# kyegomez/Tree-Attention-Torch

Hardware: NVIDIA B200
Metric: attention fwd tokens/sec (decode step Sq=1: KV tokens attended per second, whole box, device-timed, max over ranks) at seq=128K (higher is better)
Workload: dtype bf16

## Files before the change

### bench_tools/trace_decode.py

```python
import argparse
import json
import os
import sys

sys.path.insert(0, os.path.dirname(os.path.dirname(os.path.abspath(__file__))))
import torch

from tree_attention_b200 import _build
from tree_attention_b200.ops import local as L


def main():
    ap = argparse.ArgumentParser()
    ap.add_argument("--seq", type=int, nargs="*", default=[16384, 32768, 65536, 131072])
    ap.add_argument("--heads", type=int, default=32)
    ap.add_argument("--dim", type=int, default=128)
    ap.add_argument("--steps", type=int, default=50)
    a = ap.parse_args()
    C = _build.load()
    dev = torch.device("cuda")
    nsm = C.num_sms()
    for S in a.seq:
        g = torch.Generator(device=dev).manual_seed(0)
        q = torch.randn(1, a.heads, 1, a.dim, device=dev, generator=g).bfloat16()
# ... 1 lines not shown
        kvs = [(torch.randn(1, a.heads, S, a.dim, device=dev, generator=g).bfloat16(),
                torch.randn(1, a.heads, S, a.dim, device=dev, generator=g).bfloat16()) for _ in range(min(nbuf, 8))]
        out = torch.empty_like(q)
        res = {"seq": S, "kv_mb": 2 * a.heads * S * a.dim * 2 / 1e6}
        for pdl in (0, 2):
            for i in range(10):
                L.decode_attention(q, *kvs[i % len(kvs)], 0.088, out=out, return_lse=False, pdl=pdl)
            torch.cuda.synchronize()
            e0, e1 = torch.cuda.Event(enable_timing=True), torch.cuda.Event(enable_timing=True)
            e0.record()
            for i in range(a.steps):
                L.decode_attention(q, *kvs[i % len(kvs)], 0.088, out=out, return_lse=False, pdl=pdl)
            e1.record()
            torch.cuda.synchronize()
            res[f"us_per_step_pdl{pdl}"] = e0.elapsed_time(e1) / a.steps * 1e3
        tr = torch.zeros(nsm * 16, dtype=torch.int64, device=dev)
        C.decode_set_trace(tr)
        L.decode_attention(q, *kvs[0], 0.088, out=out, return_lse=False)
        torch.cuda.synchronize()
        tr.zero_()
        e0, e1 = torch.cuda.Event(enable_timing=True), torch.cuda.Event(enable_timing=True)
        e0.record()
        L.decode_attention(q, *kvs[1 % len(kvs)], 0.088, out=out, return_lse=False)
        e1.record()
        torch.cuda.synchronize()
        C.decode_set_trace(None)
        t = tr.view(nsm, 16).cpu().double()
        t = t[t[:, 0] > 0]
        g0 = t[:, 0].min()
        cyc = (t[:, 8] - t[:, 1])
        ns = (t[:, 9] - t[:, 0])
        mhz = float((cyc / ns).median() * 1e3)
        res["traced_kernel_us_event"] = e0.elapsed_time(e1) * 1e3
        res["sm_mhz_from_stamps"] = mhz

        def stat(x):
            x = x.sort().values
            return [round(float(v), 2) for v in (x[0], x[len(x) // 2], x[-1])]

        us = lambda c: c / mhz
        res["cta_start_skew_us(min,med,max)"] = stat((t[:, 0] - g0) / 1e3)
        res["prologue_us"] = stat(us(t[:, 2] - t[:, 1]))
        res["entry_to_first_tma_issue_us"] = stat(us(t[:, 10] - t[:, 1]))
        res["entry_to_first_tile_landed_us"] = stat(us(t[:, 4] - t[:, 1]))
        res["stream_first_tile_to_last_consumed_us"] = stat(us(t[:, 5] - t[:, 4]))
        res["last_finalize_us"] = stat(us(t[:, 6] - t[:, 5]))
        res["drain_us"] = stat(us(t[:, 8] - t[:, 6]))
        res["cta_total_us"] = stat(ns / 1e3)
        res["kernel_span_us(first entry -> last end)"] = float((t[:, 9].max() - g0) / 1e3)
        res["tiles_per_cta"] = stat(t[:, 12])
        res["producer_issue_span_us"] = stat(us(t[:, 11] - t[:, 10]))
        per_tile = us(t[:, 5] - t[:, 4]) / (t[:, 12] - 1).clamp(min=1)
        res["us_per_tile"] = stat(per_tile)
        sw = t[t[:, 14] > 0]
        if len(sw):
            fin = (sw[:, 14].long() & 0xffffffff).double()
            ldq = (sw[:, 14].long() >> 32).double()
            wt = (sw[:, 15].long() & 0xffffffff).double()
            pos = (sw[:, 15].long() >> 32).double()
            res["switch_finalize_us"] = stat(us(fin))
            res["switch_load_q_us"] = stat(us(ldq))
            res["switch_wait_next_tile_us"] = stat(us(wt))
            res["switch_tile_index"] = stat(pos)
            before = us(sw[:, 7] - sw[:, 4]) / pos.clamp(min=1)
            after = us(sw[:, 5] - sw[:, 7]) / (sw[:, 12] - pos).clamp(min=1)
            res["switch_cta_us_per_tile_before"] = stat(before)
            res["switch_cta_us_per_tile_after"] = stat(after)
        if os.environ.get("TRACE_DUMP"):
            torch.save(t, os.path.join(os.environ["TRACE_DUMP"], f"trace_{S}.pt"))
        print(json.dumps(res), flush=True)
        del kvs


if __name__ == "__main__":
    main()
```

### tree_attention_b200/csrc/bindings.cpp

```cpp
#include <ATen/cuda/CUDAContext.h>
#include <c10/cuda/CUDAGuard.h>
#include <pybind11/stl.h>
#include <torch/extension.h>

#include <cstring>

#include "host_utils.h"
#include "kernels.h"

namespace py = pybind11;
using ta::AttnShape;
using ta::CommCtxHost;

namespace {

py::tuple symm_alloc(int64_t nbytes) {
  void* p = nullptr;
  TA_CUDA_CHECK(cudaMalloc(&p, (size_t)nbytes));
  TA_CUDA_CHECK(cudaMemset(p, 0, (size_t)nbytes));
  TA_CUDA_CHECK(cudaDeviceSynchronize());
  cudaIpcMemHandle_t h;
  TA_CUDA_CHECK(cudaIpcGetMemHandle(&h, p));
  return py::make_tuple((int64_t) reinterpret_cast<uintptr_t>(p),
                        py::bytes(reinterpret_cast<const char*>(&h), sizeof(h)));
}
int64_t symm_open(const std::string& handle) {
  if (handle.size() != sizeof(cudaIpcMemHandle_t)) throw std::runtime_error("symm_open: bad handle size");
  cudaIpcMemHandle_t h;
  std::memcpy(&h, handle.data(), sizeof(h));
  void* p = nullptr;
  TA_CUDA_CHECK(cudaIpcOpenMemHandle(&p, h, cudaIpcMemLazyEnablePeerAccess));
  return (int64_t) reinterpret_cast<uintptr_t>(p);
}
void symm_close(int64_t ptr) { TA_CUDA_CHECK(cudaIpcCloseMemHandle(reinterpret_cast<void*>(ptr))); }
void symm_free(int64_t ptr) { TA_CUDA_CHECK(cudaFree(reinterpret_cast<void*>(ptr))); }
void symm_memset(int64_t ptr, int value, int64_t nbytes) {
  TA_CUDA_CHECK(cudaMemsetAsync(reinterpret_cast<void*>(ptr), value, (size_t)nbytes,
                                at::cuda::getCurrentCUDAStream()));
}
std::vector<uint32_t> symm_read_u32(int64_t ptr, int n) {
  std::vector<uint32_t> v(n);
  TA_CUDA_CHECK(cudaMemcpy(v.data(), reinterpret_cast<void*>(ptr), n * sizeof(uint32_t), cudaMemcpyDeviceToHost));
  return v;
}

struct Comm {
  CommCtxHost h;
  Comm(int rank, int world, std::vector<int64_t> data, std::vector<int64_t> flags, int64_t epoch, int64_t status,
       int64_t data_bytes, int64_t flag_bytes, double timeout_s) {
    if (world > ta::kMaxWorldHost) throw std::runtime_error("world size > 16 not supported");
    if ((int)data.size() != world || (int)flags.size() != world) throw std::runtime_error("Comm: pointer table size");
    h.rank = rank;
    h.world = world;
    for (int i = 0; i < world; ++i) {
      h.data[i] = reinterpret_cast<void*>(data[i]);
      h.flags[i] = reinterpret_cast<void*>(flags[i]);
    }
    h.epoch = reinterpret_cast<void*>(epoch);
    h.status = reinterpret_cast<void*>(status);
// ... 3 lines not shown
  }
};

AttnShape make_shape(const at::Tensor& q, const at::Tensor& k, const at::Tensor& v, const at::Tensor& out,
                     double scale, bool causal, int64_t q_pos0, int64_t kv_pos0, bool host_io = false) {
  TORCH_CHECK(k.is_cuda() && v.is_cuda(), "k and v must be CUDA tensors");
  TORCH_CHECK((q.is_cuda() || (host_io && q.is_pinned())) && (out.is_cuda() || (host_io && out.is_pinned())),
              host_io ? "q / out must be CUDA or pinned host tensors" : "tensors must be CUDA");
  TORCH_CHECK(q.dim() == 4 && k.dim() == 4 && v.dim() == 4 && out.dim() == 4, "expected (B, H, S, D) tensors");
  TORCH_CHECK(q.scalar_type() == at::kBFloat16 || q.scalar_type() == at::kHalf, "q must be bf16 or fp16");
  TORCH_CHECK(k.scalar_type() == q.scalar_type() && v.scalar_type() == q.scalar_type() &&
                  out.scalar_type() == q.scalar_type(), "q, k, v, out must share a dtype");
  TORCH_CHECK(q.stride(3) == 1 && k.stride(3) == 1 && v.stride(3) == 1 && out.stride(3) == 1,
              "head_dim must be contiguous");
  TORCH_CHECK(k.sizes() == v.sizes(), "k and v shapes differ");
  TORCH_CHECK(q.size(0) == k.size(0) && q.size(3) == k.size(3), "batch / head_dim mismatch");
  TORCH_CHECK(out.sizes() == q.sizes(), "out must have q's shape");
  AttnShape s;
  s.B = (int)q.size(0); s.Hq = (int)q.size(1); s.Sq = (int)q.size(2); s.D = (int)q.size(3);
  s.Hkv = (int)k.size(1); s.S = (int)k.size(2);
  s.is_bf16 = q.scalar_type() == at::kBFloat16;
  s.softmax_scale = (float)scale;
  s.causal = causal;
  s.q_pos0 = q_pos0; s.kv_pos0 = kv_pos0;
  s.q_sb = q.stride(0); s.q_sh = q.stride(1); s.q_ss = q.stride(2);
  s.k_sb = k.stride(0); s.k_sh = k.stride(1); s.k_ss = k.stride(2);
  s.v_sb = v.stride(0); s.v_sh = v.stride(1); s.v_ss = v.stride(2);
  s.o_sb = out.stride(0); s.o_sh = out.stride(1); s.o_ss = out.stride(2);
  return s;
}

const int* kv_len_ptr(const c10::optional<at::Tensor>& kv_len, const at::Tensor& like) {
  if (!kv_len.has_value()) return nullptr;
  TORCH_CHECK(kv_len->is_cuda() && kv_len->device() == like.device() && kv_len->scalar_type() == at::kInt && kv_len->numel() == 1,
              "kv_len must be a 1-element int32 CUDA tensor on the KV cache's device");
  return kv_len->data_ptr<int>();
}

py::tuple decode_plan(int B, int Hq, int Hkv, int Sq, int S, int D) {
  AttnShape s;
  s.B = B; s.Hq = Hq; s.Hkv = Hkv; s.Sq = Sq; s.S = S; s.D = D;
  int grid, mp, R;
  size_t pf, cf, cfl;
  ta::decode_simt_plan(s, ta::num_sms(), &grid, &mp, &R, &pf, &cf, &cfl);
  return py::make_tuple(grid, mp, R, (int64_t)pf, (int64_t)cf, (int64_t)cfl);
}

void decode_fwd(const at::Tensor& q, const at::Tensor& k, const at::Tensor& v, at::Tensor& out,
                c10::optional<at::Tensor> lse, at::Tensor& part, at::Tensor& tickets, py::object comm, double scale,
                bool causal, int64_t q_pos0, int64_t kv_pos0, int pdl, c10::optional<at::Tensor> kv_len) {
  c10::cuda::CUDAGuard guard(q.device());
  AttnShape s = make_shape(q, k, v, out, scale, causal, q_pos0, kv_pos0);
  TORCH_CHECK(part.scalar_type() == at::kFloat && part.is_contiguous(), "part must be contiguous fp32");
  TORCH_CHECK(tickets.scalar_type() == at::kInt && tickets.numel() >= s.B * s.Hkv + 2, "tickets too small");
  int grid, mp, R;
  size_t pf, cf, cfl;
  ta::decode_simt_plan(s, ta::num_sms(), &grid, &mp, &R, &pf, &cf, &cfl);
  TORCH_CHECK((size_t)part.numel() >= pf, "part workspace too small: need ", pf, " floats");
  float* lse_p = nullptr;
  if (lse.has_value()) {
    TORCH_CHECK(lse->scalar_type() == at::kFloat && lse->is_contiguous() && lse->numel() == (int64_t)s.B * s.Hq * s.Sq,
                "lse must be contiguous fp32 (B, Hq, Sq)");
    lse_p = lse->data_ptr<float>();
  }
  CommCtxHost c;
  if (!comm.is_none()) c = comm.cast<Comm&>().h;
  ta::decode_simt_launch(s, q.data_ptr(), k.data_ptr(), v.data_ptr(), out.data_ptr(), lse_p, part.data_ptr<float>(),
                         reinterpret_cast<uint32_t*>(tickets.data_ptr<int>()), c, ta::num_sms(),
                         at::cuda::getCurrentCUDAStream(), nullptr, nullptr, pdl, kv_len_ptr(kv_len, k));
}

py::tuple attn_fwd_comm_bytes(int B, int Hq, int Sq, int D, int world, int comm_mode) {
  AttnShape s;
  s.B = B; s.Hq = Hq; s.Sq = Sq; s.D = D;
  size_t fb = 0;
  size_t db = ta::attn_fwd_comm_bytes(s, world, &fb, comm_mode);
  return py::make_tuple((int64_t)db, (int64_t)fb);
}

void attn_fwd(const at::Tensor& q, const at::Tensor& k, const at::Tensor& v, at::Tensor& out, at::Tensor& lse,
              double scale, bool causal, int64_t q_pos0, int64_t kv_pos0, py::object comm, int variant, int comm_mode,
              int64_t kv_seg_len, int64_t kv_seg_gap) {
  c10::cuda::CUDAGuard guard(q.device());
  const bool sharded = !comm.is_none() && comm_mode == 2;
  AttnShape s = make_shape(q, k, v, sharded ? q : out, scale, causal, q_pos0, kv_pos0);
  s.kv_seg_len = (int)kv_seg_len; s.kv_seg_gap = kv_seg_gap;
  int64_t sq_out = s.Sq;
  if (sharded) {
    TORCH_CHECK(out.dim() == 4 && out.is_cuda() && out.scalar_type() == q.scalar_type() && out.stride(3) == 1 &&
                    out.size(0) == q.size(0) && out.size(1) == q.size(1) && out.size(3) == q.size(3),
                "sharded out must be (B, Hq, sq_out, D) in q's dtype");
    sq_out = out.size(2);
    const int world = comm.cast<Comm&>().h.world;
    const int64_t num_m = (s.Sq + 127) / 128;
    TORCH_CHECK(sq_out == (num_m + world - 1) / world * 128, "sharded out must have ceil(ceil(Sq/128)/world)*128 rows");
    s.o_sb = out.stride(0); s.o_sh = out.stride(1); s.o_ss = out.stride(2);
  }
  TORCH_CHECK(lse.scalar_type() == at::kFloat && lse.is_contiguous() && lse.numel() == (int64_t)s.B * s.Hq * sq_out,
              "lse must be contiguous fp32 (B, Hq, Sq) [(B, Hq, sq_out) for a sharded output]");
  CommCtxHost c;
  if (!comm.is_none()) c = comm.cast<Comm&>().h;
  TORCH_CHECK(variant == 0 || variant == 1 || variant == 6, "attn_fwd: unknown variant ", variant);
  ta::attn_fwd_launch(s, q.data_ptr(), k.data_ptr(), v.data_ptr(), out.data_ptr(), lse.data_ptr<float>(), c,
                      at::cuda::getCurrentCUDAStream(), variant == 6 ? 1 : 0, comm_mode, (int)sq_out);
}

py::tuple decode_tc_plan(int B, int Hq, int Hkv, int Sq, int S, int D) {
// ... 85 lines not shown
  TORCH_CHECK(ksc.scalar_type() == at::kFloat && vsc.scalar_type() == at::kFloat && ksc.is_contiguous() && vsc.is_contiguous() &&
                  ksc.numel() == k8.size(0) * k8.size(1) * 128 && vsc.numel() == ksc.numel(), "scales must be fp32 (B, Hkv, 128)");
  TORCH_CHECK(q.stride(2) % 8 == 0 || q.size(2) == 1, "q rows must be 16-byte aligned");
  AttnShape s;
  s.B = (int)q.size(0); s.Hq = (int)q.size(1); s.Sq = (int)q.size(2); s.D = 128;
  s.Hkv = (int)k8.size(1); s.S = (int)k8.size(2);
  s.is_bf16 = q.scalar_type() == at::kBFloat16;
  s.softmax_scale = (float)scale; s.causal = causal; s.q_pos0 = q_pos0; s.kv_pos0 = kv_pos0;
  s.q_sb = q.stride(0); s.q_sh = q.stride(1); s.q_ss = q.stride(2);
  s.k_sb = k8.stride(0); s.k_sh = k8.stride(1); s.k_ss = k8.stride(2);
  s.v_sb = v8.stride(0); s.v_sh = v8.stride(1); s.v_ss = v8.stride(2);
  s.o_sb = out.stride(0); s.o_sh = out.stride(1); s.o_ss = out.stride(2);
  int grid, mp, R;
  size_t pf, cb;
  ta::decode_tc_plan(s, ta::num_sms(), &grid, &mp, &R, &pf, &cb);
  TORCH_CHECK((size_t)part.numel() >= pf && tickets.numel() >= s.B * s.Hkv + 2, "workspace too small");
  float* lse_p = lse.has_value() ? lse->data_ptr<float>() : nullptr;
  CommCtxHost c;
  if (!comm.is_none()) c = comm.cast<Comm&>().h;
  if (swap)
    ta::decode_swap_launch(s, q.data_ptr(), k8.data_ptr(), v8.data_ptr(), out.data_ptr(), lse_p, part.data_ptr<float>(),
                           reinterpret_cast<uint32_t*>(tickets.data_ptr<int>()), c, ta::num_sms(), at::cuda::getCurrentCUDAStream(),
                           ksc.data_ptr<float>(), vsc.data_ptr<float>(), nullptr, nullptr, kv_len_ptr(kv_len, k8));
  else
    ta::decode_tc_launch(s, q.data_ptr(), k8.data_ptr(), v8.data_ptr(), out.data_ptr(), lse_p, part.data_ptr<float>(),
                         reinterpret_cast<uint32_t*>(tickets.data_ptr<int>()), c, ta::num_sms(), at::cuda::getCurrentCUDAStream(),
                         ksc.data_ptr<float>(), vsc.data_ptr<float>(), kv_len_ptr(kv_len, k8));
}

void decode_fwd_mx(const at::Tensor& q, const at::Tensor& k8, const at::Tensor& v8, const at::Tensor& ks,
                   const at::Tensor& vs, at::Tensor& out, c10::optional<at::Tensor> lse, at::Tensor& part,
                   at::Tensor& tickets, py::object comm, double scale, bool causal, int64_t q_pos0, int64_t kv_pos0,
                   c10::optional<at::Tensor> kv_len) {
  c10::cuda::CUDAGuard guard(q.device());
  TORCH_CHECK(q.dim() == 4 && k8.dim() == 4 && v8.dim() == 4 && out.sizes() == q.sizes(), "expected (B, H, S, D) tensors");
  TORCH_CHECK(q.scalar_type() == at::kBFloat16 || q.scalar_type() == at::kHalf, "q must be bf16 or fp16");
  TORCH_CHECK(out.scalar_type() == q.scalar_type() && q.stride(3) == 1 && out.stride(3) == 1);
  TORCH_CHECK(k8.scalar_type() == at::kByte && v8.scalar_type() == at::kByte && k8.stride(3) == 1 && v8.stride(3) == 1);
  TORCH_CHECK(k8.sizes() == v8.sizes() && k8.size(3) == 128 && q.size(3) == 128, "mxfp8 decode needs head_dim 128");
  TORCH_CHECK(ks.scalar_type() == at::kByte && vs.scalar_type() == at::kByte && ks.is_contiguous() && vs.is_contiguous() &&
                  ks.numel() == k8.numel() / 32 && vs.numel() == v8.numel() / 32, "scales must be contiguous uint8 (B, Hkv, S, 4)");
  AttnShape s;
  s.B = (int)q.size(0); s.Hq = (int)q.size(1); s.Sq = (int)q.size(2); s.D = 128;
  s.Hkv = (int)k8.size(1); s.S = (int)k8.size(2);
  s.is_bf16 = q.scalar_type() == at::kBFloat16;
  s.softmax_scale = (float)scale; s.causal = causal; s.q_pos0 = q_pos0; s.kv_pos0 = kv_pos0;
  s.q_sb = q.stride(0); s.q_sh = q.stride(1); s.q_ss = q.stride(2);
  s.k_sb = k8.stride(0); s.k_sh = k8.stride(1); s.k_ss = k8.stride(2);
  s.v_sb = v8.stride(0); s.v_sh = v8.stride(1); s.v_ss = v8.stride(2);
  s.o_sb = out.stride(0); s.o_sh = out.stride(1); s.o_ss = out.stride(2);
  int grid, mp, R;
  size_t pf, cf, cfl;
  ta::decode_simt_plan(s, ta::num_sms(), &grid, &mp, &R, &pf, &cf, &cfl);
  TORCH_CHECK((size_t)part.numel() >= pf && tickets.numel() >= s.B * s.Hkv + 2, "workspace too small");
  float* lse_p = lse.has_value() ? lse->data_ptr<float>() : nullptr;
  CommCtxHost c;
  if (!comm.is_none()) c = comm.cast<Comm&>().h;
  ta::decode_simt_launch(s, q.data_ptr(), k8.data_ptr(), v8.data_ptr(), out.data_ptr(), lse_p, part.data_ptr<float>(),
                         reinterpret_cast<uint32_t*>(tickets.data_ptr<int>()), c, ta::num_sms(),
                         at::cuda::getCurrentCUDAStream(), reinterpret_cast<const uint32_t*>(ks.data_ptr()),
                         reinterpret_cast<const uint32_t*>(vs.data_ptr()), 0, kv_len_ptr(kv_len, k8));
}

struct DecodeStep {
  ta::PreparedLaunch launches[3];
  bool has[3] = {false, false, false};
  std::vector<at::Tensor> keep;
  py::object comm_keep;
  c10::Device device;
  int kernels_per_step = 1;
  std::string impl;

  explicit DecodeStep(c10::Device d) : device(d) {}

  void launch(int pdl) {
    c10::cuda::CUDAGuard guard(device);
    if (pdl < 0 || pdl > 2 || !has[pdl]) pdl = 0;
    launches[pdl].run(at::cuda::getCurrentCUDAStream());
  }
};

void* io_ptr(const at::Tensor& t) {
  if (t.is_cuda()) return t.data_ptr();
  void* d = nullptr;
  const cudaError_t e = cudaHostGetDevicePointer(&d, t.data_ptr(), 0);
  TORCH_CHECK(e == cudaSuccess && d != nullptr, "pinned host tensor is not mapped into the device address space: ", cudaGetErrorString(e));
  return d;
}

std::shared_ptr<DecodeStep> decode_step(const std::string& impl, const at::Tensor& q, const at::Tensor& k, const at::Tensor& v,
                                        at::Tensor& out, c10::optional<at::Tensor> lse, at::Tensor& part, at::Tensor& tickets,
                                        py::object comm, double scale, bool causal, int64_t q_pos0, int64_t kv_pos0,
                                        c10::optional<at::Tensor> kv_len) {
  c10::cuda::CUDAGuard guard(k.device());
  AttnShape s = make_shape(q, k, v, out, scale, causal, q_pos0, kv_pos0, true);
  TORCH_CHECK(part.scalar_type() == at::kFloat && part.is_contiguous(), "part must be contiguous fp32");
  TORCH_CHECK(tickets.scalar_type() == at::kInt && tickets.numel() >= s.B * s.Hkv + 2, "tickets too small");
  float* lse_p = nullptr;
  if (lse.has_value()) {
    TORCH_CHECK(lse->scalar_type() == at::kFloat && lse->is_contiguous() && lse->numel() == (int64_t)s.B * s.Hq * s.Sq,
                "lse must be contiguous fp32 (B, Hq, Sq)");
    lse_p = lse->data_ptr<float>();
  }
  CommCtxHost c;
  if (!comm.is_none()) c = comm.cast<Comm&>().h;
  auto st = std::make_shared<DecodeStep>(k.device());
  st->impl = impl;
  st->comm_keep = comm;
  st->keep = {q, k, v, out, part, tickets};
  if (lse.has_value()) st->keep.push_back(*lse);
  if (kv_len.has_value()) st->keep.push_back(*kv_len);
  const int* kvl = kv_len_ptr(kv_len, k);
  uint32_t* tk = reinterpret_cast<uint32_t*>(tickets.data_ptr<int>());
  if (impl == "simt") {
    int grid, mp, R;
    size_t pf, cf, cfl;
    ta::decode_simt_plan(s, ta::num_sms(), &grid, &mp, &R, &pf, &cf, &cfl);
    TORCH_CHECK((size_t)part.numel() >= pf, "part workspace too small: need ", pf, " floats");
    for (int pdl = 0; pdl < 3; ++pdl) {
      st->launches[pdl] = ta::decode_simt_prepare(s, io_ptr(q), k.data_ptr(), v.data_ptr(), io_ptr(out), lse_p,
                                                  part.data_ptr<float>(), tk, c, ta::num_sms(), nullptr, nullptr, pdl, kvl);
      st->has[pdl] = true;
    }
    st->kernels_per_step = (int)st->launches[0].passes.size();
  } else if (impl == "swap" || impl == "tc") {
    int grid, mp, R;
    size_t pf, cb;
    ta::decode_tc_plan(s, ta::num_sms(), &grid, &mp, &R, &pf, &cb);
    TORCH_CHECK((size_t)part.numel() >= pf, "part workspace too small: need ", pf, " floats");
    TORCH_CHECK(q.stride(2) % 8 == 0 || q.size(2) == 1, "q rows must be 16-byte aligned");
    st->launches[0] = impl == "swap"
                          ? ta::decode_swap_prepare(s, io_ptr(q), k.data_ptr(), v.data_ptr(), io_ptr(out), lse_p,
                                                    part.data_ptr<float>(), tk, c, ta::num_sms(), nullptr, nullptr, nullptr, nullptr, kvl)
                          : ta::decode_tc_prepare(s, io_ptr(q), k.data_ptr(), v.data_ptr(), io_ptr(out), lse_p,
                                                  part.data_ptr<float>(), tk, c, ta::num_sms(), nullptr, nullptr, kvl);
    st->has[0] = true;
  } else {
    TORCH_CHECK(false, "decode_step: impl must be 'simt', 'swap' or 'tc'");
  }
  return st;
}

py::tuple quant_mxfp8(const at::Tensor& x) {
  c10::cuda::CUDAGuard guard(x.device());
  TORCH_CHECK(x.is_cuda() && x.is_contiguous() && x.size(-1) % 32 == 0, "x must be contiguous with last dim % 32 == 0");
  int dt = x.scalar_type() == at::kBFloat16 ? 0 : x.scalar_type() == at::kHalf ? 1 : 2;
  TORCH_CHECK(dt != 2 || x.scalar_type() == at::kFloat, "x must be bf16, fp16 or fp32");
  auto q = at::empty(x.sizes(), x.options().dtype(at::kByte));
  auto sizes = x.sizes().vec();
  sizes.back() /= 32;
  auto sc = at::empty(sizes, x.options().dtype(at::kByte));
  ta::quant_mxfp8_launch(x.data_ptr(), dt, q.data_ptr<uint8_t>(), sc.data_ptr<uint8_t>(), x.numel() / 32,
                         at::cuda::getCurrentCUDAStream());
  return py::make_tuple(q, sc);
}

py::tuple quant_mxfp8_seq(const at::Tensor& x) {
  c10::cuda::CUDAGuard guard(x.device());
  TORCH_CHECK(x.is_cuda() && x.is_contiguous() && x.dim() == 4 && x.size(3) % 32 == 0, "x must be contiguous (B, H, S, D), D % 32 == 0");
  int dt = x.scalar_type() == at::kBFloat16 ? 0 : x.scalar_type() == at::kHalf ? 1 : 2;
  TORCH_CHECK(dt != 2 || x.scalar_type() == at::kFloat, "x must be bf16, fp16 or fp32");
  const int64_t B = x.size(0), H = x.size(1), S = x.size(2), D = x.size(3), T = (S + 127) / 128;
  auto q = at::empty(x.sizes(), x.options().dtype(at::kByte));
  auto sc = at::empty({B, H, T, D, 4}, x.options().dtype(at::kByte));
  ta::quant_mxfp8_seq_launch(x.data_ptr(), dt, q.data_ptr<uint8_t>(), sc.data_ptr<uint8_t>(), B * H, (int)S, (int)D,
                             at::cuda::getCurrentCUDAStream());
  return py::make_tuple(q, sc);
}

void mxfp8_seq_append(at::Tensor& data, at::Tensor& sc, const at::Tensor& x, int64_t position) {
  c10::cuda::CUDAGuard guard(data.device());
// ... 117 lines not shown
  m.def("decode_fwd", &decode_fwd, py::arg("q"), py::arg("k"), py::arg("v"), py::arg("out"), py::arg("lse"), py::arg("part"),
        py::arg("tickets"), py::arg("comm"), py::arg("scale"), py::arg("causal"), py::arg("q_pos0"), py::arg("kv_pos0"),
        py::arg("pdl") = 0, py::arg("kv_len") = py::none());
  m.def("decode_fwd_mx", &decode_fwd_mx, py::arg("q"), py::arg("k8"), py::arg("v8"), py::arg("ks"), py::arg("vs"), py::arg("out"),
        py::arg("lse"), py::arg("part"), py::arg("tickets"), py::arg("comm"), py::arg("scale"), py::arg("causal"),
        py::arg("q_pos0"), py::arg("kv_pos0"), py::arg("kv_len") = py::none());
  m.def("decode_set_trace", [](c10::optional<at::Tensor> t) {
    if (!t.has_value()) { ta::decode_simt_set_trace(nullptr); return; }
    TORCH_CHECK(t->is_cuda() && t->scalar_type() == at::kLong && t->is_contiguous() && t->numel() >= 16 * ta::num_sms());
    ta::decode_simt_set_trace(reinterpret_cast<unsigned long long*>(t->data_ptr<int64_t>()));
  });
  m.def("decode_tc_plan", &decode_tc_plan);
  m.def("decode_tc_fwd", &decode_tc_fwd, py::arg("q"), py::arg("k"), py::arg("v"), py::arg("out"), py::arg("lse"), py::arg("part"),
        py::arg("tickets"), py::arg("comm"), py::arg("scale"), py::arg("causal"), py::arg("q_pos0"), py::arg("kv_pos0"),
        py::arg("swap"), py::arg("kv_len") = py::none());
  m.def("decode_tc_fwd8", &decode_tc_fwd8, py::arg("q"), py::arg("k8"), py::arg("v8"), py::arg("ksc"), py::arg("vsc"), py::arg("out"),
        py::arg("lse"), py::arg("part"), py::arg("tickets"), py::arg("comm"), py::arg("scale"), py::arg("causal"),
        py::arg("q_pos0"), py::arg("kv_pos0"), py::arg("swap"), py::arg("kv_len") = py::none());
  m.def("decode_mx_tc_fwd", &decode_mx_tc_fwd, py::arg("q"), py::arg("k8"), py::arg("v8"), py::arg("k_sf"), py::arg("v_sf"),
        py::arg("out"), py::arg("lse"), py::arg("part"), py::arg("tickets"), py::arg("comm"), py::arg("scale"), py::arg("causal"),
        py::arg("q_pos0"), py::arg("kv_pos0"), py::arg("kv_len") = py::none());
  py::class_<DecodeStep, std::shared_ptr<DecodeStep>>(m, "DecodeStep")
      .def("launch", &DecodeStep::launch, py::arg("pdl") = 0)
      .def_readonly("kernels_per_step", &DecodeStep::kernels_per_step)
      .def_readonly("impl", &DecodeStep::impl);
  m.def("decode_step", &decode_step, py::arg("impl"), py::arg("q"), py::arg("k"), py::arg("v"), py::arg("out"), py::arg("lse"),
        py::arg("part"), py::arg("tickets"), py::arg("comm"), py::arg("scale"), py::arg("causal"), py::arg("q_pos0"),
        py::arg("kv_pos0"), py::arg("kv_len") = py::none());
  m.def("quant_mxfp8", &quant_mxfp8);
  m.def("quant_mxfp8_seq", &quant_mxfp8_seq);
  m.def("mxfp8_seq_append", &mxfp8_seq_append);
  m.def("dequant_mxfp8", &dequant_mxfp8);
  m.def("attn_fwd", &attn_fwd, py::arg("q"), py::arg("k"), py::arg("v"), py::arg("out"), py::arg("lse"), py::arg("scale"),
        py::arg("causal"), py::arg("q_pos0"), py::arg("kv_pos0"), py::arg("comm"), py::arg("variant") = 0, py::arg("comm_mode") = 1,
        py::arg("kv_seg_len") = 0, py::arg("kv_seg_gap") = 0);
  m.def("attn_fwd_comm_bytes", &attn_fwd_comm_bytes, py::arg("B"), py::arg("Hq"), py::arg("Sq"), py::arg("D"), py::arg("world"),
        py::arg("comm_mode") = 1);
  m.def("attn_fwd_phase_cycles", []() { unsigned long long c[5]; ta::attn_fwd_phase_cycles(c); return py::make_tuple(c[0], c[1], c[2], c[3], c[4]); });
  m.def("attn_bwd", &attn_bwd);
  m.def("symm_allreduce", &symm_allreduce);
  m.def("symm_allreduce_sizes", &symm_allreduce_sizes);
  m.def("combine", &combine);
  m.def("umma_probe", &umma_probe);
  m.def("umma_bs_probe", &umma_bs_probe, py::arg("a8"), py::arg("b8"), py::arg("sfa"), py::arg("sfb"), py::arg("c"),
        py::arg("a_mn_major") = false);
  m.def("umma_2cta_probe", [](const at::Tensor& a, const at::Tensor& b, at::Tensor& c) {
    c10::cuda::CUDAGuard guard(a.device());
    TORCH_CHECK(a.scalar_type() == at::kBFloat16 && b.scalar_type() == at::kBFloat16 && c.scalar_type() == at::kFloat);
    TORCH_CHECK(a.is_contiguous() && b.is_contiguous() && c.is_contiguous() && a.size(0) == 256 && a.size(1) == 64 &&
                b.size(0) == 128 && b.size(1) == 64 && c.size(0) == 256 && c.size(1) == 128);
    ta::umma_2cta_probe_launch(a.data_ptr(), b.data_ptr(), c.data_ptr<float>(), 128, at::cuda::getCurrentCUDAStream());
  });
  m.def("num_sms", []() { return ta::num_sms(); });
  m.def("decode_split_for", [](int B, int Hkv, int S, int ncta) {
    AttnShape s{};
    s.B = B; s.Hkv = Hkv; s.Hq = Hkv; s.Sq = 1; s.S = S; s.D = 128;
    int g = 0, mp = 0;
    ta::decode_split(B * Hkv, S, ncta, &g, &mp);
    return py::make_tuple(g, mp);
  });
  m.def("tmem_ld_bw_probe", [](int warps, int iters) { return ta::tmem_ld_bw_probe(warps, iters, at::cuda::getCurrentCUDAStream()); });
}
```

### tree_attention_b200/csrc/common.cuh

```cuda
#pragma once
#include <cuda.h>
#include <cuda_bf16.h>
#include <cuda_fp16.h>
#include <cuda_runtime.h>
#include <stdint.h>
#include <stdio.h>

namespace ta {

#ifndef TA_SPIN_TIMEOUT_NS
#define TA_SPIN_TIMEOUT_NS 4000000000ull
#endif

constexpr int kMaxWorld = 16;

__device__ __forceinline__ uint32_t smem_u32(const void* p) {
  return static_cast<uint32_t>(__cvta_generic_to_shared(p));
}
__device__ __forceinline__ uint64_t globaltimer_ns() {
  uint64_t t;
  asm volatile("mov.u64 %0, %%globaltimer;" : "=l"(t));
  return t;
}
__device__ __forceinline__ uint32_t lane_id() { return threadIdx.x & 31; }
// ... 62 lines not shown
__device__ __forceinline__ float bf16lo(uint32_t w) { return __uint_as_float(w << 16); }
__device__ __forceinline__ float bf16hi(uint32_t w) { return __uint_as_float(w & 0xffff0000u); }
__device__ __forceinline__ uint32_t pack_bf16x2(float lo, float hi) {
  uint32_t r;
  asm("cvt.rn.bf16x2.f32 %0, %1, %2;" : "=r"(r) : "f"(hi), "f"(lo));
  return r;
}
__device__ __forceinline__ uint32_t pack_f16x2(float lo, float hi) {
  uint32_t r;
  asm("cvt.rn.f16x2.f32 %0, %1, %2;" : "=r"(r) : "f"(hi), "f"(lo));
  return r;
}
__device__ __forceinline__ float f16lo(uint32_t w) {
  return __half2float(__ushort_as_half(static_cast<unsigned short>(w & 0xffffu)));
}
__device__ __forceinline__ float f16hi(uint32_t w) {
  return __half2float(__ushort_as_half(static_cast<unsigned short>(w >> 16)));
}

__device__ __forceinline__ uint64_t pack_f32x2(float a, float b) {
  uint64_t r;
  asm("mov.b64 %0, {%1, %2};" : "=l"(r) : "f"(a), "f"(b));
  return r;
}
__device__ __forceinline__ void unpack_f32x2(uint64_t v, float& a, float& b) {
  asm("mov.b64 {%0, %1}, %2;" : "=f"(a), "=f"(b) : "l"(v));
}
__device__ __forceinline__ uint64_t fma2_f32x2(uint64_t a, uint64_t b, uint64_t c) {
  uint64_t d;
  asm("fma.rn.f32x2 %0, %1, %2, %3;" : "=l"(d) : "l"(a), "l"(b), "l"(c));
  return d;
}
__device__ __forceinline__ uint64_t add2_f32x2(uint64_t a, uint64_t b) {
  uint64_t d;
  asm("add.rn.f32x2 %0, %1, %2;" : "=l"(d) : "l"(a), "l"(b));
  return d;
}

__device__ __forceinline__ void mbar_init(uint64_t* bar, uint32_t count) {
  asm volatile("mbarrier.init.shared::cta.b64 [%0], %1;" ::"r"(smem_u32(bar)), "r"(count) : "memory");
}
__device__ __forceinline__ void fence_mbar_init() {
  asm volatile("fence.mbarrier_init.release.cluster;" ::: "memory");
}
__device__ __forceinline__ void fence_proxy_async_smem() {
  asm volatile("fence.proxy.async.shared::cta;" ::: "memory");
}
__device__ __forceinline__ void mbar_arrive(uint64_t* bar) {
  asm volatile("mbarrier.arrive.shared::cta.b64 _, [%0];" ::"r"(smem_u32(bar)) : "memory");
}
__device__ __forceinline__ void mbar_arrive_expect_tx(uint64_t* bar, uint32_t bytes) {
  asm volatile("mbarrier.arrive.expect_tx.shared::cta.b64 _, [%0], %1;" ::"r"(smem_u32(bar)), "r"(bytes)
               : "memory");
}
__device__ __forceinline__ bool mbar_try_wait(uint64_t* bar, uint32_t parity) {
  uint32_t ok;
  asm volatile(
      "{\n\t.reg .pred P;\n\t"
      "mbarrier.try_wait.parity.shared::cta.b64 P, [%1], %2;\n\t"
      "selp.u32 %0, 1, 0, P;\n\t}"
      : "=r"(ok)
      : "r"(smem_u32(bar)), "r"(parity)
      : "memory");
  return ok != 0;
}
__device__ __forceinline__ void mbar_wait(uint64_t* bar, uint32_t parity) {
  if (mbar_try_wait(bar, parity)) return;
  uint64_t t0 = globaltimer_ns();
  uint32_t it = 0;
  while (!mbar_try_wait(bar, parity)) {
    if ((++it & 0x3ffu) == 0 && globaltimer_ns() - t0 > TA_SPIN_TIMEOUT_NS) {
      printf("[tree_attention] mbarrier wait timeout block=(%d,%d) thread=%d bar=%u parity=%u\n",
             blockIdx.x, blockIdx.y, threadIdx.x, smem_u32(bar), parity);
      __trap();
    }
  }
}

__device__ __forceinline__ void tma_prefetch_desc(const CUtensorMap* m) {
  asm volatile("prefetch.tensormap [%0];" ::"l"(reinterpret_cast<uint64_t>(m)) : "memory");
}
__device__ __forceinline__ void tma_load_4d(void* smem_dst, const CUtensorMap* map, uint64_t* bar,
                                            int c0, int c1, int c2, int c3) {
  asm volatile(
      "cp.async.bulk.tensor.4d.shared::cluster.global.mbarrier::complete_tx::bytes [%0], [%1, {%3, %4, %5, %6}], [%2];"
      ::"r"(smem_u32(smem_dst)), "l"(reinterpret_cast<uint64_t>(map)), "r"(smem_u32(bar)), "r"(c0), "r"(c1),
      "r"(c2), "r"(c3)
      : "memory");
}
__device__ __forceinline__ void tma_load_2d(void* smem_dst, const CUtensorMap* map, uint64_t* bar,
                                            int c0, int c1) {
  asm volatile(
      "cp.async.bulk.tensor.2d.shared::cluster.global.mbarrier::complete_tx::bytes [%0], [%1, {%3, %4}], [%2];"
      ::"r"(smem_u32(smem_dst)), "l"(reinterpret_cast<uint64_t>(map)), "r"(smem_u32(bar)), "r"(c0), "r"(c1)
      : "memory");
}
__device__ __forceinline__ void tma_store_4d(const CUtensorMap* map, const void* smem_src, int c0, int c1,
                                             int c2, int c3) {
  asm volatile(
      "cp.async.bulk.tensor.4d.global.shared::cta.bulk_group [%0, {%2, %3, %4, %5}], [%1];"
      ::"l"(reinterpret_cast<uint64_t>(map)), "r"(smem_u32(smem_src)), "r"(c0), "r"(c1), "r"(c2), "r"(c3)
      : "memory");
}
__device__ __forceinline__ void tma_store_commit() { asm volatile("cp.async.bulk.commit_group;" ::: "memory"); }
template <int N>
__device__ __forceinline__ void tma_store_wait_read() {
// ... 213 lines not shown
```

### tree_attention_b200/csrc/decode_comm.cuh

```cuda
#pragma once
#include "common.cuh"
#include "kernels.h"

namespace ta {
namespace dcomm {

constexpr int kTileKeys = 128;
constexpr int kPartChunk = 8;

__device__ __forceinline__ float ninf() { return __int_as_float(0xff800000); }

struct Geom {
  int S;
  int tph;
  int total;
  int tiles_q, tiles_rem;
};

__device__ __forceinline__ Geom make_geom(int cap, const int* kv_len, int BH, int ncta) {
  Geom g;
  int s = cap;
  if (kv_len != nullptr) s = max(0, min(cap, *reinterpret_cast<const volatile int*>(kv_len)));
  g.S = s;
  g.tph = max(1, (s + kTileKeys - 1) / kTileKeys);
  g.total = BH * g.tph;
  g.tiles_q = g.total / ncta;
  g.tiles_rem = g.total - g.tiles_q * ncta;
  return g;
}
__device__ __forceinline__ int cta_lo(const Geom& g, int c) { return c * g.tiles_q + min(c, g.tiles_rem); }
__device__ __forceinline__ int cta_of_tile(const Geom& g, int t) {
  const int big = g.tiles_rem * (g.tiles_q + 1);
  return t < big ? t / (g.tiles_q + 1) : g.tiles_rem + (t - big) / max(g.tiles_q, 1);
}

__device__ __forceinline__ void ll_store_sys(uint64_t* w, float v, uint32_t tag) {
  const uint64_t x = ((uint64_t)tag << 32) | (uint64_t)__float_as_uint(v);
  asm volatile("st.relaxed.sys.global.u64 [%0], %1;" ::"l"(w), "l"(x) : "memory");
}
__device__ __forceinline__ uint64_t ll_load_sys(const uint64_t* w) {
  uint64_t r;
  asm volatile("ld.relaxed.sys.global.u64 %0, [%1];" : "=l"(r) : "l"(w) : "memory");
  return r;
}
__device__ __forceinline__ void ll_store_gpu(uint64_t* w, float v, uint32_t tag) {
  const uint64_t x = ((uint64_t)tag << 32) | (uint64_t)__float_as_uint(v);
  asm volatile("st.relaxed.gpu.global.u64 [%0], %1;" ::"l"(w), "l"(x) : "memory");
}
__device__ __forceinline__ uint64_t ll_load_gpu(const uint64_t* w) {
  uint64_t r;
  asm volatile("ld.relaxed.gpu.global.u64 %0, [%1];" : "=l"(r) : "l"(w) : "memory");
  return r;
}
__device__ __forceinline__ uint32_t ll_tag(uint64_t w) { return (uint32_t)(w >> 32); }
__device__ __forceinline__ float ll_val(uint64_t w) { return __uint_as_float((uint32_t)w); }

static __device__ __noinline__ uint64_t ll_spin_sys(const uint64_t* w, uint32_t tag, unsigned long long timeout_ns) {
  const uint64_t t0 = globaltimer_ns();
  uint32_t it = 0;
  uint64_t out;
  while (true) {
    out = ll_load_sys(w);
    if (ll_tag(out) == tag) break;
    if ((++it & 0x3fu) == 0 && globaltimer_ns() - t0 > timeout_ns) break;
  }
  return out;
}
static __device__ __noinline__ uint64_t ll_spin_gpu(const uint64_t* w, uint32_t tag) {
  const uint64_t t0 = globaltimer_ns();
  uint32_t it = 0;
  uint64_t out;
  while (true) {
    out = ll_load_gpu(w);
    if (ll_tag(out) == tag) break;
    if ((++it & 0x3fu) == 0 && globaltimer_ns() - t0 > TA_SPIN_TIMEOUT_NS) {
      printf("[tree_attention] split-merge wait timeout block=%d thread=%d tag=%u\n", blockIdx.x, threadIdx.x, tag);
      __trap();
    }
  }
  return out;
}

constexpr int kTagShift = 12;

__device__ __forceinline__ uint32_t launch_tag(unsigned long long* ctr) {
  const unsigned long long inc = blockIdx.x == 0 ? (unsigned long long)((1u << kTagShift) - (gridDim.x - 1)) : 1ull;
  const unsigned long long old = atomicAdd(ctr, inc);
  return (uint32_t)(old >> kTagShift) + 1u;
}

struct Tail {
  const CommCtx* comm;
  uint64_t* part;
  int max_parts;
  int BH;
  int R;
  int rows_valid;
  uint32_t wtag;
  uint32_t ctag;
  Geom geo;
  int* pending;
  int max_pending;
  uint64_t* stamps;
};

template <int D>
__device__ __forceinline__ uint64_t* part_ptr(const Tail& t, int x, int pidx) {
  return t.part + ((size_t)x * t.max_parts + pidx) * (size_t)(t.R * (D + 2));
}
template <int D>
__device__ __forceinline__ uint64_t* word_ptr(const Tail& t, int dst, int src, int x) {
  return reinterpret_cast<uint64_t*>(t.comm->data[dst]) +
         ((size_t)((t.ctag & 1) * t.comm->world + src) * t.BH + x) * (size_t)(t.R * (D + 2));
}
__device__ __forceinline__ void head_parts(const Geom& g, int x, int cta, int& nparts, int& pidx) {
  const int first_cta = cta_of_tile(g, x * g.tph);
  nparts = cta_of_tile(g, (x + 1) * g.tph - 1) - first_cta + 1;
  pidx = cta - first_cta;
}

template <int D>
__device__ __forceinline__ void merge_parts(const Tail& t, int x, int nparts, int r, int d, float& o_norm, float& lse2) {
  const size_t pstride = (size_t)t.R * (D + 2);
  const uint64_t* base = part_ptr<D>(t, x, 0) + (size_t)r * (D + 2);
  float M = ninf(), acc = 0.f, L = 0.f;
  for (int q0 = 0; q0 < nparts; q0 += kPartChunk) {
    uint64_t wa[kPartChunk], wm[kPartChunk], wl[kPartChunk];
#pragma unroll
    for (int i = 0; i < kPartChunk; ++i) {
      if (q0 + i < nparts) {
        const uint64_t* pp = base + (size_t)(q0 + i) * pstride;
        wa[i] = ll_load_gpu(pp + d); wm[i] = ll_load_gpu(pp + D); wl[i] = ll_load_gpu(pp + D + 1);
      }
    }
    float m[kPartChunk], a[kPartChunk], l[kPartChunk];
    float Mn = M;
#pragma unroll
    for (int i = 0; i < kPartChunk; ++i) {
      m[i] = ninf(); a[i] = 0.f; l[i] = 0.f;
      if (q0 + i < nparts) {
        const uint64_t* pp = base + (size_t)(q0 + i) * pstride;
        if (ll_tag(wa[i]) != t.wtag) wa[i] = ll_spin_gpu(pp + d, t.wtag);
        if (ll_tag(wm[i]) != t.wtag) wm[i] = ll_spin_gpu(pp + D, t.wtag);
        if (ll_tag(wl[i]) != t.wtag) wl[i] = ll_spin_gpu(pp + D + 1, t.wtag);
        a[i] = ll_val(wa[i]); m[i] = ll_val(wm[i]); l[i] = ll_val(wl[i]);
        Mn = fmaxf(Mn, m[i]);
      }
    }
    const float Ms = (Mn == ninf()) ? 0.f : Mn;
    const float sc0 = fast_exp2(M - Ms);
    acc *= sc0; L *= sc0;
#pragma unroll
    for (int i = 0; i < kPartChunk; ++i) {
      const float sc = fast_exp2(m[i] - Ms);
      acc = fmaf(a[i], sc, acc);
      L = fmaf(l[i], sc, L);
    }
    M = Mn;
  }
  const float Ms = (M == ninf()) ? 0.f : M;
  o_norm = L > 0.f ? acc / L : 0.f;
  lse2 = L > 0.f ? Ms + fast_log2(L) : ninf();
}

template <int D>
__device__ __forceinline__ void publish(const Tail& t, int x, int r, int d, float o_norm, float lse2) {
  const int world = t.comm->world;
#pragma unroll 4
  for (int dst = 0; dst < world; ++dst) {
    uint64_t* wp = word_ptr<D>(t, dst, t.comm->rank, x) + r * (D + 2);
    ll_store_sys(wp + d, o_norm, t.ctag);
    if (d == 0) ll_store_sys(wp + D, lse2, t.ctag);
  }
}

template <int D, int RB>
__device__ __forceinline__ bool gather_rows(const Tail& t, int x, int r0, int nr, int d, float (&o_norm)[RB],
                                            float (&lse2)[RB], int& bad_src) {
  constexpr int kSrcChunk = RB >= 4 ? 4 : 8;
  const int world = t.comm->world;
  const size_t src_stride = (size_t)t.BH * t.R * (D + 2);
  const uint64_t* w0 = word_ptr<D>(t, t.comm->rank, 0, x);
  float m_run[RB], num[RB], den[RB];
#pragma unroll
  for (int i = 0; i < RB; ++i) { m_run[i] = ninf(); num[i] = 0.f; den[i] = 0.f; }
  bool ok = true;
  for (int s0 = 0; s0 < world; s0 += kSrcChunk) {
    uint64_t lw[RB][kSrcChunk], vw[RB][kSrcChunk];
#pragma unroll
    for (int i = 0; i < RB; ++i) {
#pragma unroll
      for (int s = 0; s < kSrcChunk; ++s) {
        if (i < nr && s0 + s < world) {
          const uint64_t* wr = w0 + (size_t)(s0 + s) * src_stride + (size_t)(r0 + i) * (D + 2);
          lw[i][s] = ll_load_sys(wr + D);
          vw[i][s] = ll_load_sys(wr + d);
        }
// ... 24 lines not shown
        for (int s = 0; s < kSrcChunk; ++s) {
          const float w = fast_exp2(ls[s] - ms);
          num[i] = fmaf(w, vs[s], num[i]);
          den[i] += w;
        }
        m_run[i] = mc;
      }
    }
  }
#pragma unroll
  for (int i = 0; i < RB; ++i) {
    const float ms = (m_run[i] == ninf()) ? 0.f : m_run[i];
    o_norm[i] = den[i] > 0.f ? num[i] / den[i] : 0.f;
    lse2[i] = den[i] > 0.f ? ms + fast_log2(den[i]) : ninf();
  }
  return ok;
}

template <int D, int NT, int RB, typename StoreOut>
__device__ __noinline__ void combine_ranks(const Tail& t, int x, int tid, int bar_id, StoreOut& store_out) {
  static_assert(NT % D == 0, "thread count must be a multiple of head_dim");
  constexpr int NG = NT / D;
  const int d = tid % D, g = tid / D;
  uint64_t t_got = 0;
  for (int r0 = g * RB; r0 < t.rows_valid; r0 += NG * RB) {
    const int nr = min(RB, t.rows_valid - r0);
    float o_norm[RB], lse2[RB];
    int bad_src = -1;
    const bool ok = gather_rows<D, RB>(t, x, r0, nr, d, o_norm, lse2, bad_src);
    if (tid == 0 && r0 == 0) t_got = globaltimer_ns();
    if (!ok) {
      t.comm->status[0] = kCommTimeout; t.comm->status[1] = x; t.comm->status[2] = bad_src; t.comm->status[3] = t.ctag;
    }
#pragma unroll
    for (int i = 0; i < RB; ++i) {
      if (i < nr) {
        const float nan = __int_as_float(0x7fc00000);
        store_out(x, r0 + i, d, ok ? o_norm[i] : nan, ok ? lse2[i] : nan);
      }
    }
  }
  if (tid == 0 && t.stamps[1] != 0) {
    const uint64_t t_done = globaltimer_ns(), t_publish = t.stamps[1], t_cta0 = t.stamps[0];
    atomicMax(t.comm->status + 10, (uint32_t)min((unsigned long long)(t_got - t_publish), 0xffffffffull));
    atomicMax(t.comm->status + 11, (uint32_t)min((unsigned long long)(t_done - t_publish), 0xffffffffull));
    atomicMax(t.comm->status + 12, (uint32_t)min((unsigned long long)(t_publish - t_cta0), 0xffffffffull));
  }
}

template <int D, int NT, typename StoreOut>
__device__ __noinline__ void merge_head(const Tail& t, int x, int tid, StoreOut& store_out) {
  static_assert(NT % D == 0, "thread count must be a multiple of head_dim");
  constexpr int NG = NT / D;
  int nparts, pidx;
  head_parts(t.geo, x, blockIdx.x, nparts, pidx);
  const int world = t.comm->world;
  const int d = tid % D;
  for (int r = tid / D; r < t.rows_valid; r += NG) {
    float o_norm, lse2;
    merge_parts<D>(t, x, nparts, r, d, o_norm, lse2);
    if (world == 1) store_out(x, r, d, o_norm, lse2);
    else if (!t.comm->skip_publish) publish<D>(t, x, r, d, o_norm, lse2);
  }
}

template <int D, int NT, int RB, typename StoreOut>
__device__ __forceinline__ void segment_done(const Tail& t, int x, int seg_end_tile, int& n_pend, int tid, int bar_id,
                                             StoreOut& store_out) {
  if (seg_end_tile != (x + 1) * t.geo.tph) return;
  if (n_pend >= t.max_pending) {
    printf("[tree_attention] pending-merge list overflow block=%d head=%d\n", blockIdx.x, x);
    __trap();
  }
  if (tid == 0) t.pending[n_pend] = x;
  ++n_pend;
}

template <int D, int NT, int RB, typename StoreOut>
__device__ __forceinline__ void drain(const Tail& t, int n_pend, int tid, int bar_id, StoreOut& store_out) {
  named_bar_sync(bar_id, NT);
  for (int i = 0; i < n_pend; ++i) merge_head<D, NT>(t, t.pending[i], tid, store_out);
  if (t.comm->world <= 1 || n_pend == 0) return;
  if (tid == 0) t.stamps[1] = globaltimer_ns();
  named_bar_sync(bar_id, NT);
  for (int i = 0; i < n_pend; ++i) combine_ranks<D, NT, RB>(t, t.pending[i], tid, bar_id, store_out);
}

inline CommCtx to_device_ctx(const CommCtxHost& h) {
  CommCtx c;
  c.rank = h.rank;
  c.world = h.world;
  for (int i = 0; i < kMaxWorld; ++i) {
    c.data[i] = reinterpret_cast<float*>(h.data[i]);
    c.flags[i] = reinterpret_cast<uint32_t*>(h.flags[i]);
  }
  c.epoch = reinterpret_cast<uint32_t*>(h.epoch);
  c.status = reinterpret_cast<uint32_t*>(h.status);
  c.timeout_ns = h.timeout_ns;
  c.skip_publish = h.skip_publish;
  return c;
}

}
}
```

### tree_attention_b200/csrc/decode_simt.cu

```cuda
#include "common.cuh"
#include "decode_comm.cuh"
#include "host_utils.h"
#include "kernels.h"

namespace ta {

namespace {

constexpr int kTileRows = 128;
constexpr int kConsumerWarps = 8;
constexpr int kConsumerThreads = kConsumerWarps * 32;
constexpr int kThreads = kConsumerThreads + 32;
constexpr int kRowsPerWarp = kTileRows / kConsumerWarps;
constexpr int kMaxPending = 64;

struct DecodeParams {
  const void* q;
  void* out;
  float* lse;
  const uint32_t* kscale;
  const uint32_t* vscale;
  uint64_t* part;
  unsigned long long* wctr;
  const int* kv_len;
  int B, Hq, Hkv, G, Sq, S;
  int rows_valid;
  int r_base;
  float scale_log2;
  int causal;
  long long q_pos0, kv_pos0;
  long long q_sb, q_sh, q_ss, o_sb, o_sh, o_ss;
  int max_parts;
  unsigned long long* trace;
  int pdl;
  CommCtx comm;
};

template <int D, bool KV8>
struct SmemLayout {
  static constexpr int kElem = KV8 ? 1 : 2;
  static constexpr int kAtoms = D * kElem / 128;
  static constexpr int kTensorBytes = kTileRows * D * kElem;
  static constexpr int kStageBytes = 2 * kTensorBytes;
  static constexpr int kStages = (D * kElem == 256) ? 3 : 6;
  static constexpr int kPsPerWarp = KV8 ? 4 : 1;
};

template <int D, int R, bool KV8>
constexpr size_t smem_bytes() {
  using L = SmemLayout<D, KV8>;
  return 1024  + size_t(L::kStages) * L::kStageBytes +
         sizeof(float) * (2 * R * D + kConsumerWarps * L::kPsPerWarp * R * kRowsPerWarp +
                          (R <= 2 ? 2 : 1) * kConsumerWarps * R * (D + 4)) +
         sizeof(int) * (kMaxPending + 8) + sizeof(uint64_t) * (2 * L::kStages + 2);
}

template <bool BF16>
__device__ __forceinline__ void cvt8(const uint4& w, float (&f)[8]) {
  if constexpr (BF16) {
    f[0] = bf16lo(w.x); f[1] = bf16hi(w.x); f[2] = bf16lo(w.y); f[3] = bf16hi(w.y);
    f[4] = bf16lo(w.z); f[5] = bf16hi(w.z); f[6] = bf16lo(w.w); f[7] = bf16hi(w.w);
  } else {
    f[0] = f16lo(w.x); f[1] = f16hi(w.x); f[2] = f16lo(w.y); f[3] = f16hi(w.y);
    f[4] = f16lo(w.z); f[5] = f16hi(w.z); f[6] = f16lo(w.w); f[7] = f16hi(w.w);
  }
}
template <bool BF16>
__device__ __forceinline__ float cvt1(uint16_t h) {
  if constexpr (BF16) return __uint_as_float(uint32_t(h) << 16);
  else return __half2float(__ushort_as_half(h));
}
template <bool BF16>
__device__ __forceinline__ uint16_t to16(float f) {
  if constexpr (BF16) return __bfloat16_as_ushort(__float2bfloat16_rn(f));
  else return __half_as_ushort(__float2half_rn(f));
}

__device__ __forceinline__ float neg_inf() { return __int_as_float(0xff800000); }

template <int D, int R, bool BF16, bool KV8>
__global__ void __launch_bounds__(kThreads, 1)
decode_simt_kernel(const __grid_constant__ CUtensorMap kmap, const __grid_constant__ CUtensorMap vmap,
                   const __grid_constant__ DecodeParams p) {
  using L = SmemLayout<D, KV8>;
  constexpr int NS = L::kStages;
  constexpr int EPL = D / 32;
  extern __shared__ uint8_t smem_raw[];
  uint8_t* smem = reinterpret_cast<uint8_t*>((reinterpret_cast<uintptr_t>(smem_raw) + 1023) & ~uintptr_t(1023));
  uint8_t* stage_base = smem;
  float* q_s = reinterpret_cast<float*>(smem + size_t(NS) * L::kStageBytes);
  float* p_s = q_s + 2 * R * D;
  float* merge_s = p_s + kConsumerWarps * L::kPsPerWarp * R * kRowsPerWarp;
  constexpr int kMergeBufs = R <= 2 ? 2 : 1;
  int* pending = reinterpret_cast<int*>(merge_s + kMergeBufs * kConsumerWarps * R * (D + 4));
  int* s_misc = pending + kMaxPending;
  uint64_t* full_bar = reinterpret_cast<uint64_t*>(s_misc + 8);
  uint64_t* empty_bar = full_bar + NS;
  uint64_t* stamps = empty_bar + NS;

  const int tid = threadIdx.x;
  const int warp = tid >> 5;
  const int lane = tid & 31;
  const int cta = blockIdx.x;
  const int world = p.comm.world;
  unsigned long long* trc = p.trace ? p.trace + (size_t)cta * 16 : nullptr;
  if (trc && tid == 0) {
    trc[0] = globaltimer_ns(); trc[1] = clock64();
    uint32_t smid;
    asm volatile("mov.u32 %0, %%smid;" : "=r"(smid));
    trc[13] = smid; trc[14] = 0; trc[15] = 0;
  }

  if (tid == 0) {
    for (int i = 0; i < NS; ++i) {
      mbar_init(&full_bar[i], 1);
      mbar_init(&empty_bar[i], kConsumerWarps);
    }
    fence_mbar_init();
    s_misc[0] = 0; s_misc[1] = 0; s_misc[6] = 0;
  }
  if (warp == kConsumerWarps && lane == 0) {
    tma_prefetch_desc(&kmap);
    tma_prefetch_desc(&vmap);
  }
  __syncthreads();
  if (trc && tid == 0) trc[2] = clock64();

  if (p.pdl) asm volatile("griddepcontrol.launch_dependents;" ::: "memory");
  const int BH = p.B * p.Hkv;
  const long long q_pos_max = p.q_pos0 + p.Sq - 1;

  auto tile_visible = [&](int j) -> bool {
    return !p.causal || (p.kv_pos0 + (long long)j * kTileRows <= q_pos_max);
  };

  if (warp == kConsumerWarps) {
    if (lane == 0) {
      if (p.pdl == 1) asm volatile("griddepcontrol.wait;" ::: "memory");
      const dcomm::Geom geo = dcomm::make_geom(p.S, p.kv_len, BH, gridDim.x);
      const int t_lo = dcomm::cta_lo(geo, cta), t_hi = dcomm::cta_lo(geo, cta + 1);
      int stage = 0, issued = 0;
      uint32_t phase = 0;
      bool tags_done = false;
      auto fetch_tags = [&]() {
        if (p.pdl == 2) asm volatile("griddepcontrol.wait;" ::: "memory");
        const uint32_t wtag = dcomm::launch_tag(p.wctr);
        const uint32_t ctag = world > 1 ? dcomm::launch_tag(reinterpret_cast<unsigned long long*>(p.comm.epoch)) : 0u;
        volatile int* sm = s_misc;
        sm[4] = (int)wtag; sm[5] = (int)ctag;
        __threadfence_block();
        sm[6] = 1;
        tags_done = true;
      };
      for (int t = t_lo; t < t_hi; ++t) {
        const int x = t / geo.tph, j = t - x * geo.tph;
        if (!tile_visible(j)) continue;
        const int b = x / p.Hkv, h = x - b * p.Hkv;
        if (issued == NS && !tags_done) fetch_tags();
        mbar_wait(&empty_bar[stage], phase ^ 1);
        if (trc && issued == 0) trc[10] = clock64();
        mbar_arrive_expect_tx(&full_bar[stage], L::kStageBytes);
        uint8_t* ks = stage_base + size_t(stage) * L::kStageBytes;
        uint8_t* vs = ks + L::kTensorBytes;
#pragma unroll
        for (int a = 0; a < L::kAtoms; ++a) {
          tma_load_4d(ks + a * (kTileRows * 128), &kmap, &full_bar[stage], a * (128 / L::kElem), j * kTileRows, h, b);
          tma_load_4d(vs + a * (kTileRows * 128), &vmap, &full_bar[stage], a * (128 / L::kElem), j * kTileRows, h, b);
        }
        ++issued;
        if (++stage == NS) { stage = 0; phase ^= 1; }
      }
      if (!tags_done) fetch_tags();
      if (trc) { trc[11] = clock64(); trc[12] = (unsigned long long)issued; }
    }
    return;
  }

  if (p.pdl) asm volatile("griddepcontrol.wait;" ::: "memory");
  if (trc && tid == 0) trc[3] = clock64();
  const dcomm::Geom geo = dcomm::make_geom(p.S, p.kv_len, BH, gridDim.x);
  const int t_lo = dcomm::cta_lo(geo, cta), t_hi = dcomm::cta_lo(geo, cta + 1);
  constexpr int RB = R;
  if (tid == 0) { stamps[0] = globaltimer_ns(); stamps[1] = 0; }
  auto make_tail = [&]() {
    dcomm::Tail tl;
    volatile int* sm = s_misc;
    while (sm[6] == 0) { }
    tl.comm = &p.comm; tl.part = p.part; tl.max_parts = p.max_parts; tl.BH = BH;
    tl.R = R; tl.rows_valid = p.rows_valid; tl.wtag = (uint32_t)sm[4]; tl.ctag = (uint32_t)sm[5]; tl.geo = geo;
    tl.pending = pending; tl.max_pending = kMaxPending; tl.stamps = stamps;
    return tl;
  };
  const int r16 = lane & 15;
  const int half = lane >> 4;
  float m_run[R], l_run[R], o_acc[R][EPL];
  int cur_x = -1;
  int stage = 0;
  uint32_t phase = 0;

  auto reset_state = [&]() {
#pragma unroll
    for (int r = 0; r < R; ++r) {
      m_run[r] = neg_inf();
      l_run[r] = 0.f;
#pragma unroll
      for (int e = 0; e < EPL; ++e) o_acc[r][e] = 0.f;
    }
  };

  auto load_q = [&](int x, int buf) {
    const int b = x / p.Hkv, h = x - b * p.Hkv;
    for (int idx = tid; idx < R * D; idx += kConsumerThreads) {
      const int r = idx / D, d = idx - r * D;
      float val = 0.f;
      if (r < p.rows_valid) {
        const int rr = p.r_base + r;
        const int g = rr / p.Sq, i = rr - g * p.Sq;
        const uint16_t* qp = reinterpret_cast<const uint16_t*>(p.q) + (long long)b * p.q_sb +
                             (long long)(h * p.G + g) * p.q_sh + (long long)i * p.q_ss + d;
        val = cvt1<BF16>(*qp) * p.scale_log2;
      }
      if constexpr (KV8) reinterpret_cast<__half*>(q_s + buf * R * D)[idx] = __float2half_rn(val);
      else q_s[buf * R * D + idx] = val;
    }
  };
  const int x_first = t_lo / geo.tph;
  if (t_lo < t_hi) {
    load_q(x_first, 0);
    if ((x_first + 1) * geo.tph < t_hi) load_q(x_first + 1, 1);
  }
  named_bar_sync(1, kConsumerThreads);
  const float* q_cur = q_s;
  uint32_t wtag = 0;
  int n_fin = 0;
  int n_pend = 0;

  auto store_out = [&](int x, int r, int d, float o_norm, float lse2) {
    const int b = x / p.Hkv, h = x - b * p.Hkv;
    const int rr = p.r_base + r;
    const int g = rr / p.Sq, i = rr - g * p.Sq;
    uint16_t* op = reinterpret_cast<uint16_t*>(p.out) + (long long)b * p.o_sb + (long long)(h * p.G + g) * p.o_sh +
                   (long long)i * p.o_ss + d;
    *op = to16<BF16>(o_norm);
    if (d == 0 && p.lse != nullptr)
      p.lse[((long long)b * p.Hq + (h * p.G + g)) * p.Sq + i] = lse2 * 0.6931471805599453f;
  };

  auto finalize_segment = [&](int x) {
    float* mbuf = merge_s + (kMergeBufs == 2 ? (n_fin & 1) : 0) * (kConsumerWarps * R * (D + 4));
    ++n_fin;
#pragma unroll
    for (int r = 0; r < R; ++r) {
      float lt = l_run[r];
      lt += __shfl_xor_sync(0xffffffffu, lt, 8);
      lt += __shfl_xor_sync(0xffffffffu, lt, 4);
      lt += __shfl_xor_sync(0xffffffffu, lt, 2);
      lt += __shfl_xor_sync(0xffffffffu, lt, 1);
      float* ms = mbuf + (warp * R + r) * (D + 4);
#pragma unroll
      for (int e = 0; e < EPL; ++e) ms[lane * EPL + e] = o_acc[r][e];
      if (lane == 0) { ms[D] = m_run[r]; ms[D + 1] = lt; }
    }
    named_bar_sync(1, kConsumerThreads);
    if (wtag == 0) {
      volatile int* sm = s_misc;
      while (sm[6] == 0) { }
      wtag = (uint32_t)sm[4];
    }
    int nparts, pidx;
    dcomm::head_parts(geo, x, cta, nparts, pidx);
    uint64_t* my_part = p.part + ((size_t)x * p.max_parts + pidx) * (size_t)(R * (D + 2));
    for (int idx = tid; idx < R * D; idx += kConsumerThreads) {
      const int r = idx / D, d = idx - r * D;
      float M = neg_inf();
#pragma unroll
      for (int w = 0; w < kConsumerWarps; ++w) M = fmaxf(M, mbuf[(w * R + r) * (D + 4) + D]);
      const float Ms = (M == neg_inf()) ? 0.f : M;
      float acc = 0.f, Lsum = 0.f;
#pragma unroll
      for (int w = 0; w < kConsumerWarps; ++w) {
        const float* ms = mbuf + (w * R + r) * (D + 4);
        const float sc = fast_exp2(ms[D] - Ms);
        acc = fmaf(ms[d], sc, acc);
        Lsum = fmaf(ms[D + 1], sc, Lsum);
      }
      dcomm::ll_store_gpu(my_part + r * (D + 2) + d, acc, wtag);
      if (d == 0) {
        dcomm::ll_store_gpu(my_part + r * (D + 2) + D, M, wtag);
        dcomm::ll_store_gpu(my_part + r * (D + 2) + D + 1, Lsum, wtag);
      }
    }
    if (min(t_hi, (x + 1) * geo.tph) == (x + 1) * geo.tph) {
      if (tid == 0) pending[n_pend] = x;
      ++n_pend;
    }
    if constexpr (kMergeBufs == 1) named_bar_sync(1, kConsumerThreads);
  };

  [[maybe_unused]] uint32_t nxt_ksc = 0, nxt_vsc = 0;
  [[maybe_unused]] auto fetch_scales = [&](int tt) {
    if constexpr (KV8) {
      if (tt < t_hi) {
        const int xx = tt / geo.tph, jj = tt - xx * geo.tph;
        const long long srow = (long long)xx * p.S + min((long long)jj * kTileRows + warp * kRowsPerWarp + (lane & 15), (long long)p.S - 1);
        nxt_ksc = __ldg(p.kscale + srow);
        nxt_vsc = __ldg(p.vscale + srow);
      }
    }
  };
  fetch_scales(t_lo);

  const uint32_t stage_a = smem_u32(stage_base);
  const uint32_t ps_a = smem_u32(p_s);
  [[maybe_unused]] uint32_t k_off[D / 16];
  [[maybe_unused]] uint32_t v_sw[8];
  [[maybe_unused]] uint32_t q_off[D / 16];
  if constexpr (!KV8) {
    const int row = warp * kRowsPerWarp + r16;
#pragma unroll
    for (int c = 0; c < D / 16; ++c) {
      const int cg = half * (D / 16) + c;
      const int atom = cg >> 3, cia = cg & 7;
      k_off[c] = uint32_t(atom * (kTileRows * 128) + row * 128 + ((cia ^ (row & 7)) << 4));
      q_off[c] = uint32_t(cg * 8 * 4);
    }
    const int c0 = lane * EPL;
    const int atom = (c0 * 2) >> 7, inner = (c0 * 2) & 127;
    const int chunk = inner >> 4, off = inner & 15;
#pragma unroll
    for (int k7 = 0; k7 < 8; ++k7)
      v_sw[k7] = uint32_t(L::kTensorBytes + atom * (kTileRows * 128) + off + ((chunk ^ k7) << 4) + (warp * kRowsPerWarp) * 128);
  }

  for (int t = t_lo; t < t_hi; ++t) {
    const int x = t / geo.tph, j = t - x * geo.tph;
    [[maybe_unused]] const uint32_t ksc_word = nxt_ksc;
    [[maybe_unused]] const uint32_t vsc_cur = nxt_vsc;
    fetch_scales(t + 1);
    bool switched = false;
    long long ts0 = 0, ts1 = 0, ts2 = 0;
    if (x != cur_x) {
      switched = cur_x >= 0;
      ts0 = clock64();
      if (cur_x >= 0) finalize_segment(cur_x);
      ts1 = clock64();
      const int rel = x - x_first;
      if (rel >= 2) {
        load_q(x, rel & 1);
        named_bar_sync(1, kConsumerThreads);
      }
      q_cur = q_s + (rel & 1) * R * D;
      reset_state();
      cur_x = x;
      ts2 = clock64();
    }
    if (!tile_visible(j)) continue;
    mbar_wait(&full_bar[stage], phase);
    if (trc && tid == 0 && t == t_lo) trc[4] = clock64();
    if (trc && tid == 0 && switched) {
      trc[14] = (unsigned long long)(ts1 - ts0) | ((unsigned long long)(ts2 - ts1) << 32);
      trc[15] = (unsigned long long)(clock64() - ts2) | ((unsigned long long)(t - t_lo) << 32);
      trc[7] = (unsigned long long)ts0;
    }
    const uint8_t* ks = stage_base + size_t(stage) * L::kStageBytes;
    const uint8_t* vs = ks + L::kTensorBytes;

    const int row = warp * kRowsPerWarp + r16;
    float s_sum[R];
    [[maybe_unused]] uint32_t vsc_word = 0;
    if constexpr (!KV8) {
      const uint32_t ks_a = stage_a + uint32_t(stage) * L::kStageBytes;
      const uint32_t q_a = smem_u32(q_cur);
      uint64_t acc2[R][2];
#pragma unroll
      for (int r = 0; r < R; ++r) { acc2[r][0] = 0ull; acc2[r][1] = 0ull; }
#pragma unroll
      for (int c = 0; c < D / 16; ++c) {
        const uint4 kw = ld_shared_v4u(ks_a + k_off[c]);
        uint64_t k2[4];
        if constexpr (BF16) {
          k2[0] = pack_f32x2(bf16lo(kw.x), bf16hi(kw.x)); k2[1] = pack_f32x2(bf16lo(kw.y), bf16hi(kw.y));
          k2[2] = pack_f32x2(bf16lo(kw.z), bf16hi(kw.z)); k2[3] = pack_f32x2(bf16lo(kw.w), bf16hi(kw.w));
        } else {
          k2[0] = pack_f32x2(f16lo(kw.x), f16hi(kw.x)); k2[1] = pack_f32x2(f16lo(kw.y), f16hi(kw.y));
          k2[2] = pack_f32x2(f16lo(kw.z), f16hi(kw.z)); k2[3] = pack_f32x2(f16lo(kw.w), f16hi(kw.w));
        }
#pragma unroll
        for (int r = 0; r < R; ++r) {
          uint64_t q01, q23, q45, q67;
          ld_shared_v2u64(q_a + uint32_t(r * D * 4) + q_off[c], q01, q23);
          ld_shared_v2u64(q_a + uint32_t(r * D * 4) + q_off[c] + 16, q45, q67);
          acc2[r][0] = fma2_f32x2(k2[0], q01, acc2[r][0]);
          acc2[r][1] = fma2_f32x2(k2[1], q23, acc2[r][1]);
          acc2[r][0] = fma2_f32x2(k2[2], q45, acc2[r][0]);
          acc2[r][1] = fma2_f32x2(k2[3], q67, acc2[r][1]);
        }
      }
#pragma unroll
      for (int r = 0; r < R; ++r) {
        float a0, a1, a2, a3;
        unpack_f32x2(acc2[r][0], a0, a1);
        unpack_f32x2(acc2[r][1], a2, a3);
        s_sum[r] = (a0 + a1) + (a2 + a3);
      }
    } else {
      vsc_word = vsc_cur;
#pragma unroll
      for (int r = 0; r < R; ++r) s_sum[r] = 0.f;
#pragma unroll
      for (int c = 0; c < 4; ++c) {
        const int cg = half * 4 + c;
        const uint4 kw = *reinterpret_cast<const uint4*>(ks + row * 128 + ((cg ^ (row & 7)) << 4));
        uint32_t kh[8];
        const uint32_t kw4[4] = {kw.x, kw.y, kw.z, kw.w};
#pragma unroll
// ... 80 lines not shown
        for (int u = 0; u < 4; ++u) {
          const int vrow = warp * kRowsPerWarp + jj + u;
          const uint32_t w = *reinterpret_cast<const uint32_t*>(vs + vrow * 128 + ((chunk ^ (vrow & 7)) << 4) + off);
          uint32_t h0, h1;
          asm("cvt.rn.f16x2.e4m3x2 %0, %1;" : "=r"(h0) : "h"((uint16_t)(w & 0xffffu)));
          asm("cvt.rn.f16x2.e4m3x2 %0, %1;" : "=r"(h1) : "h"((uint16_t)(w >> 16)));
          const float2 v01 = __half22float2(*reinterpret_cast<const __half2*>(&h0));
          const float2 v23 = __half22float2(*reinterpret_cast<const __half2*>(&h1));
#pragma unroll
          for (int r = 0; r < R; ++r) {
            const float pp = (u == 0) ? pr[r].x : (u == 1) ? pr[r].y : (u == 2) ? pr[r].z : pr[r].w;
            o_acc[r][0] = fmaf(pp, v01.x, o_acc[r][0]);
            o_acc[r][1] = fmaf(pp, v01.y, o_acc[r][1]);
            o_acc[r][2] = fmaf(pp, v23.x, o_acc[r][2]);
            o_acc[r][3] = fmaf(pp, v23.y, o_acc[r][3]);
          }
        }
      }
    } else
    {
      const uint32_t vs_a = stage_a + uint32_t(stage) * L::kStageBytes;
#pragma unroll
      for (int jj = 0; jj < kRowsPerWarp; jj += 4) {
        float4 pr[R];
#pragma unroll
        for (int r = 0; r < R; ++r) pr[r] = ld_shared_v4f(ps_a + uint32_t(((warp * R + r) * kRowsPerWarp + jj) * 4));
#pragma unroll
        for (int u = 0; u < 4; ++u) {
          const uint32_t va = vs_a + v_sw[(jj + u) & 7] + uint32_t((jj + u) * 128);
          float vf[EPL];
          if constexpr (EPL == 4) {
            const uint2 w = ld_shared_v2u(va);
            if constexpr (BF16) { vf[0] = bf16lo(w.x); vf[1] = bf16hi(w.x); vf[2] = bf16lo(w.y); vf[3] = bf16hi(w.y); }
            else { vf[0] = f16lo(w.x); vf[1] = f16hi(w.x); vf[2] = f16lo(w.y); vf[3] = f16hi(w.y); }
          } else {
            const uint32_t w = ld_shared_u32(va);
            if constexpr (BF16) { vf[0] = bf16lo(w); vf[1] = bf16hi(w); }
            else { vf[0] = f16lo(w); vf[1] = f16hi(w); }
          }
#pragma unroll
          for (int r = 0; r < R; ++r) {
            const float pp = (u == 0) ? pr[r].x : (u == 1) ? pr[r].y : (u == 2) ? pr[r].z : pr[r].w;
#pragma unroll
            for (int e = 0; e < EPL; ++e) o_acc[r][e] = fmaf(pp, vf[e], o_acc[r][e]);
          }
        }
      }
    }
    __syncwarp();
    if (lane == 0) mbar_arrive(&empty_bar[stage]);
    if (++stage == NS) { stage = 0; phase ^= 1; }
  }
  if (trc && tid == 0) trc[5] = clock64();
  if (cur_x >= 0) finalize_segment(cur_x);
  if (trc && tid == 0) trc[6] = clock64();

  const dcomm::Tail tail = make_tail();
  dcomm::drain<D, kConsumerThreads, RB>(tail, n_pend, tid, 1, store_out);
  if (trc && tid == 0) { trc[8] = clock64(); trc[9] = globaltimer_ns(); }
}

template <int D, int R, bool BF16, bool KV8>
std::function<void(cudaStream_t)> make_pass(const CUtensorMap& kmap, const CUtensorMap& vmap, const DecodeParams& p, int grid) {
  auto kern = decode_simt_kernel<D, R, BF16, KV8>;
  constexpr size_t smem = smem_bytes<D, R, KV8>();
  static bool configured = false;
  if (!configured) {
    TA_CUDA_CHECK(cudaFuncSetAttribute(kern, cudaFuncAttributeMaxDynamicSharedMemorySize, (int)smem));
    configured = true;
  }
  return [kern, kmap, vmap, p, grid](cudaStream_t stream) {
    cudaLaunchConfig_t cfg{};
    cfg.gridDim = dim3(grid);
    cfg.blockDim = dim3(kThreads);
    cfg.dynamicSmemBytes = smem_bytes<D, R, KV8>();
    cfg.stream = stream;
    cudaLaunchAttribute attr[1];
    attr[0].id = cudaLaunchAttributeProgrammaticStreamSerialization;
    attr[0].val.programmaticStreamSerializationAllowed = 1;
    cfg.attrs = attr;
    cfg.numAttrs = p.pdl ? 1 : 0;
    TA_CUDA_CHECK(cudaLaunchKernelEx(&cfg, kern, kmap, vmap, p));
  };
}

int pick_rows(int total_rows) { return total_rows >= 4 ? 4 : (total_rows >= 2 ? 2 : 1); }

unsigned long long* g_decode_trace = nullptr;

}

void decode_simt_set_trace(unsigned long long* buf) { g_decode_trace = buf; }

void decode_split(int BH, int cap, int ncta, int* grid, int* max_parts) {
  const int tph = std::max(1, (cap + kTileRows - 1) / kTileRows);
  const long long total = (long long)BH * tph;
  const int g = (int)std::min<long long>(ncta, total);
  const int mp = std::min<long long>(g, (2LL * g + BH - 1) / BH + 1);
  *grid = g;
  *max_parts = std::max(mp, 1);
}

void decode_simt_plan(const AttnShape& s, int nsm, int* grid, int* max_parts, int* rows_per_pass,
                      size_t* part_floats, size_t* comm_floats, size_t* comm_flags) {
  const int BH = s.B * s.Hkv;
  decode_split(BH, s.S, nsm, grid, max_parts);
  const int R = pick_rows((s.Hq / s.Hkv) * s.Sq);
  *rows_per_pass = R;
  *part_floats = (size_t)BH * *max_parts * R * (s.D + 2) * 2;
  *comm_floats = (size_t)2 * kMaxWorldHost * BH * R * (s.D + 2) * 2;
  *comm_flags = (size_t)2 * kMaxWorldHost * BH;
}

PreparedLaunch decode_simt_prepare(const AttnShape& s, const void* q, const void* k, const void* v, void* out, float* lse,
                                   float* part, uint32_t* tickets, const CommCtxHost& comm, int nsm,
                                   const uint32_t* kscale, const uint32_t* vscale, int pdl, const int* kv_len) {
  if ((reinterpret_cast<uintptr_t>(part) | reinterpret_cast<uintptr_t>(tickets)) & 7)
    throw std::runtime_error("decode_simt: workspace must be 8-byte aligned");
  const bool kv8 = kscale != nullptr;
  if (s.D != 64 && s.D != 128) throw std::runtime_error("decode_simt: head_dim must be 64 or 128");
  if (kv8 && s.D != 128) throw std::runtime_error("decode_simt(mxfp8): head_dim must be 128");
  if (s.Hq % s.Hkv != 0) throw std::runtime_error("decode_simt: Hq must be a multiple of Hkv");
  if (s.S <= 0) throw std::runtime_error("decode_simt: the KV shard must have capacity for at least one row");
  int grid, max_parts, R;
  size_t pf, cf, cfl;
  decode_simt_plan(s, nsm, &grid, &max_parts, &R, &pf, &cf, &cfl);
  const int G = s.Hq / s.Hkv;
  const int total_rows = G * s.Sq;
  if ((long long)s.B * s.Hkv / grid + 2 > kMaxPending)
    throw std::runtime_error("decode_simt: batch x kv-heads too large for one launch (split the batch)");
  if (comm.world > 1) {
    const size_t need_data = (size_t)2 * comm.world * s.B * s.Hkv * R * (s.D + 2) * 8;
    if (need_data > comm.data_bytes)
      throw std::runtime_error("decode_simt: symmetric buffer too small for this problem");
  }
  const int eb = kv8 ? 1 : 2;
  CUtensorMap kmap = make_tmap_bhsd(k, eb, s.B, s.Hkv, s.S, s.D, s.k_sb, s.k_sh, s.k_ss, 128 / eb, kTileRows,
                                    CU_TENSOR_MAP_SWIZZLE_128B);
  CUtensorMap vmap = make_tmap_bhsd(v, eb, s.B, s.Hkv, s.S, s.D, s.v_sb, s.v_sh, s.v_ss, 128 / eb, kTileRows,
                                    CU_TENSOR_MAP_SWIZZLE_128B);
  DecodeParams p;
  p.kscale = kscale; p.vscale = vscale; p.pdl = pdl; p.kv_len = kv_len; p.trace = g_decode_trace;
  p.q = q; p.out = out; p.lse = lse;
  p.part = reinterpret_cast<uint64_t*>(part); p.wctr = reinterpret_cast<unsigned long long*>(tickets);
  p.B = s.B; p.Hq = s.Hq; p.Hkv = s.Hkv; p.G = G; p.Sq = s.Sq; p.S = s.S;
  p.scale_log2 = s.softmax_scale * 1.4426950408889634f;
  p.causal = s.causal; p.q_pos0 = s.q_pos0; p.kv_pos0 = s.kv_pos0;
  p.q_sb = s.q_sb; p.q_sh = s.q_sh; p.q_ss = s.q_ss; p.o_sb = s.o_sb; p.o_sh = s.o_sh; p.o_ss = s.o_ss;
  p.max_parts = max_parts;
  p.comm = dcomm::to_device_ctx(comm);
  PreparedLaunch pl;
  for (int r_base = 0; r_base < total_rows; r_base += R) {
    p.r_base = r_base;
    p.rows_valid = std::min(R, total_rows - r_base);
#define TA_PASS(DD, RR, KV)                                                                       \
  pl.passes.push_back(s.is_bf16 ? make_pass<DD, RR, true, KV>(kmap, vmap, p, grid)               \
                                : make_pass<DD, RR, false, KV>(kmap, vmap, p, grid));
    if (kv8) {
      if (R == 4) { TA_PASS(128, 4, true) } else if (R == 2) { TA_PASS(128, 2, true) } else { TA_PASS(128, 1, true) }
    } else if (s.D == 128) {
      if (R == 4) { TA_PASS(128, 4, false) } else if (R == 2) { TA_PASS(128, 2, false) } else { TA_PASS(128, 1, false) }
    } else {
      if (R == 4) { TA_PASS(64, 4, false) } else if (R == 2) { TA_PASS(64, 2, false) } else { TA_PASS(64, 1, false) }
    }
#undef TA_PASS
  }
  return pl;
}

void decode_simt_launch(const AttnShape& s, const void* q, const void* k, const void* v, void* out, float* lse,
                        float* part, uint32_t* tickets, const CommCtxHost& comm, int nsm, cudaStream_t stream,
                        const uint32_t* kscale, const uint32_t* vscale, int pdl, const int* kv_len) {
  decode_simt_prepare(s, q, k, v, out, lse, part, tickets, comm, nsm, kscale, vscale, pdl, kv_len).run(stream);
}

}
```

### tree_attention_b200/csrc/decode_swap_sm100.cu

```cuda
#include "common.cuh"
#include "decode_comm.cuh"
#include "host_utils.h"
#include "kernels.h"

namespace ta {
namespace {

constexpr int kSwN = 16;
constexpr int kSwKV = 128;
constexpr int kSwD = 128;
constexpr int kSwThreads = 192;
constexpr int kSmx = 128;
constexpr int kSwMaxPending = 32;
constexpr float kSwRescale = 8.0f;
constexpr uint32_t kSfK = 96;
constexpr uint32_t kSfV = 104;
constexpr uint32_t kSfQ = 112;
constexpr uint32_t kSfP = 116;
constexpr uint32_t kSfOne = 0x7f7f7f7fu;

struct DecodeSwParams {
  const void* q;
  void* out;
  float* lse;
// ... 25 lines not shown
  static constexpr int kPBytes = kSwN * kSwKV * kElem;
  static constexpr int kPAtoms = kSwKV * kElem / 128;
  static constexpr int kStages = KV8 ? 6 : 3;
  static constexpr size_t kTotal = 1024 + size_t(2 * kStages) * kTileBytes + kQBytes + 2 * kPBytes + 2048 + 1024;
};

__device__ __forceinline__ float sw_ninf() { return __int_as_float(0xff800000); }
template <bool BF16>
__device__ __forceinline__ uint16_t sw_to16(float f) {
  if constexpr (BF16) return __bfloat16_as_ushort(__float2bfloat16_rn(f));
  else return __half_as_ushort(__float2half_rn(f));
}
__device__ __forceinline__ int sw_f2ord(float f) { const int i = __float_as_int(f); return i ^ ((i >> 31) & 0x7fffffff); }
__device__ __forceinline__ float sw_ord2f(int i) { return __int_as_float(i ^ ((i >> 31) & 0x7fffffff)); }

template <bool BF16, bool KV8, bool MX>
__global__ void __launch_bounds__(kSwThreads, 1)
decode_swap_kernel(const __grid_constant__ CUtensorMap kmap, const __grid_constant__ CUtensorMap vmap,
                   const __grid_constant__ DecodeSwParams p) {
  using SM = SwSmem<KV8>;
  constexpr int D = kSwD;
  constexpr int NS = SM::kStages;
  constexpr int EPA = 128 / SM::kElem;
  constexpr int KSTEP = 32 / SM::kElem;
  extern __shared__ uint8_t smem_raw[];
  uint8_t* smem = reinterpret_cast<uint8_t*>((reinterpret_cast<uintptr_t>(smem_raw) + 1023) & ~uintptr_t(1023));
  uint8_t* k_s = smem;
  uint8_t* v_s = k_s + NS * SM::kTileBytes;
  uint8_t* q_s = v_s + NS * SM::kTileBytes;
  uint8_t* p_s = q_s + SM::kQBytes;
  float* xch = reinterpret_cast<float*>(p_s + 2 * SM::kPBytes);
  float* red_s = xch + 2 * 4 * kSwN;
  uint64_t* bars = reinterpret_cast<uint64_t*>(red_s + 4 * kSwN);
  uint64_t* q_ready = bars;
  uint64_t* k_full = bars + 1;
  uint64_t* k_empty = k_full + NS;
  uint64_t* v_full = k_empty + NS;
  uint64_t* v_empty = v_full + NS;
  uint64_t* s_full = v_empty + NS;
  uint64_t* p_full = s_full + 2;
  uint64_t* pv_done = p_full + 2;
  uint64_t* stamps = pv_done + 2;
  uint32_t* tmem_slot = reinterpret_cast<uint32_t*>(stamps + 2);
  int* s_misc = reinterpret_cast<int*>(tmem_slot + 2);
  int* s_tags = s_misc + 4;
  int* pending = s_tags + 4;
  [[maybe_unused]] float* ch_scale = reinterpret_cast<float*>(pending + kSwMaxPending);

  const int tid = threadIdx.x, warp = tid >> 5, lane = tid & 31;
  const int cta = blockIdx.x;
  const int world = p.comm.world;
  const int BH = p.B * p.Hkv;
  const int R = p.R;
  const dcomm::Geom geo = dcomm::make_geom(p.S, p.kv_len, BH, gridDim.x);
  const int t_lo = dcomm::cta_lo(geo, cta), t_hi = dcomm::cta_lo(geo, cta + 1);
  int jvis = geo.tph;
  if (p.causal) {
    const long long last = p.q_pos0 + p.Sq - 1 - p.kv_pos0;
    jvis = (int)max(0LL, min((long long)geo.tph, last < 0 ? 0LL : last / kSwKV + 1));
  }

  if (tid == 0) {
    mbar_init(q_ready, kSmx);
    for (int i = 0; i < NS; ++i) { mbar_init(&k_full[i], 1); mbar_init(&k_empty[i], 1); mbar_init(&v_full[i], 1); mbar_init(&v_empty[i], 1); }
    for (int i = 0; i < 2; ++i) { mbar_init(&s_full[i], 1); mbar_init(&p_full[i], 4); mbar_init(&pv_done[i], 1); }
    fence_mbar_init();
    s_misc[0] = 0; s_misc[1] = 0; s_tags[2] = 0;
  }
  if (warp == 4 && lane == 0) { tma_prefetch_desc(&kmap); tma_prefetch_desc(&vmap); }
  if (warp == 5) tmem_alloc<128>(tmem_slot);
  if (warp < 4) {
    for (int c = tid; c < (SM::kQBytes + 2 * SM::kPBytes) / 16; c += kSmx) reinterpret_cast<uint4*>(q_s)[c] = make_uint4(0, 0, 0, 0);
  }
  tc_fence_before();
  __syncthreads();
  tc_fence_after();
  const uint32_t tmem = *tmem_slot;
  const uint32_t tmem_o = tmem + 64;

  if (tid == 0) { stamps[0] = globaltimer_ns(); stamps[1] = 0; }

  auto next_segment = [&](int t, int& x, int& j0, int& n, int& t_next) {
    x = t / geo.tph;
    const int seg_end = min(t_hi, (x + 1) * geo.tph);
    j0 = t - x * geo.tph;
    const int j1 = seg_end - x * geo.tph;
    n = max(0, min(j1, jvis) - j0);
    t_next = seg_end;
  };

  if (warp == 4) {
    if (lane == 0) {
      int it = 0;
      bool tags_done = false;
      auto fetch_tags = [&]() {
        const uint32_t wtag = dcomm::launch_tag(p.wctr);
        const uint32_t ctag = world > 1 ? dcomm::launch_tag(reinterpret_cast<unsigned long long*>(p.comm.epoch)) : 0u;
        volatile int* sm = s_tags;
        sm[0] = (int)wtag; sm[1] = (int)ctag;
        __threadfence_block();
        sm[2] = 1;
        tags_done = true;
      };
      for (int t = t_lo; t < t_hi;) {
        int x, j0, n, tn;
        next_segment(t, x, j0, n, tn);
        const int b = x / p.Hkv, h = x - b * p.Hkv;
// ... 55 lines not shown
        if (n > 0) {
          issue_qk(it);
          for (int jj = 0; jj < n; ++jj) {
            const int i = it + jj;
            if (jj + 1 < n) issue_qk(i + 1);
            const int st = i % NS;
            mbar_wait(&p_full[i & 1], (i >> 1) & 1);
            mbar_wait(&v_full[st], (i / NS) & 1);
            tc_fence_after();
            const uint64_t v_desc = umma_smem_desc_sw128(smem_u32(v_s + st * SM::kTileBytes), SM::kAtomBytes, 1024);
            const uint64_t pt_desc = pt_desc0 + (((i & 1) * SM::kPBytes) >> 4);
            if (leader) {
#pragma unroll
              for (int kk = 0; kk < kSwKV / KSTEP; ++kk) {
                const uint64_t ad = v_desc + ((kk * (KSTEP * 128)) >> 4);
                const uint64_t bd = pt_desc + (((kk / 4) * SM::kQAtomBytes + (kk % 4) * 32) >> 4);
                if constexpr (MX)
                  umma_ss_mxf8_block_scale(tmem_o, ad, bd, umma_idesc_block_scaled(0, 0, D, kSwN, 1, 0, kk, kk),
                                           tmem + kSfV + 4 * (i & 1), tmem + kSfP, (jj > 0 || kk > 0) ? 1u : 0u);
                else if constexpr (KV8) umma_ss_f8(tmem_o, ad, bd, idesc_pv, (jj > 0 || kk > 0) ? 1u : 0u);
                else umma_ss_f16(tmem_o, ad, bd, idesc_pv, (jj > 0 || kk > 0) ? 1u : 0u);
              }
              umma_commit(&v_empty[st]);
              umma_commit(&pv_done[i & 1]);
            }
            __syncwarp();
          }
          it += n;
        }
        ++seg;
        t = tn;
      }
    }
    __syncwarp();
  } else {
    const int row = tid;
    const uint32_t lane_addr = uint32_t(warp * 32) << 16;
    int qi_of[kSwN];
#pragma unroll
    for (int qn = 0; qn < kSwN; ++qn) qi_of[qn] = qn % p.Sq;
    auto store_out = [&](int x, int r, int d, float o_norm, float lse2) {
      const int b = x / p.Hkv, h = x - b * p.Hkv;
      const int g = r / p.Sq, i = r - g * p.Sq;
      uint16_t* op = reinterpret_cast<uint16_t*>(p.out) + (long long)b * p.o_sb + (long long)(h * p.G + g) * p.o_sh +
                     (long long)i * p.o_ss + d;
      *op = sw_to16<BF16>(o_norm);
      if (d == 0 && p.lse != nullptr) p.lse[((long long)b * p.Hq + (h * p.G + g)) * p.Sq + i] = lse2 * 0.6931471805599453f;
    };
    int n_pend = 0;
    auto make_tail = [&]() {
      dcomm::Tail tl;
      volatile int* sm = s_tags;
      while (sm[2] == 0) { }
      tl.comm = &p.comm; tl.part = p.part; tl.max_parts = p.max_parts; tl.BH = BH;
      tl.R = R; tl.rows_valid = R; tl.wtag = (uint32_t)sm[0]; tl.ctag = (uint32_t)sm[1]; tl.geo = geo;
      tl.pending = pending; tl.max_pending = kSwMaxPending; tl.stamps = stamps;
      return tl;
    };

    const uint32_t xch_a = smem_u32(xch), pt_a = smem_u32(p_s);
    [[maybe_unused]] uint32_t* sfq_s = reinterpret_cast<uint32_t*>(ch_scale);
    [[maybe_unused]] auto load_ksf = [&](int x, int j, uint32_t (&w)[4]) {
#pragma unroll
      for (int c = 0; c < 4; ++c) {
        const int key = j * kSwKV + 32 * c + lane;
        w[c] = key < p.S ? __ldg(p.k_sf + (long long)x * p.S + key) : kSfOne;
      }
    };
    [[maybe_unused]] auto load_vsf = [&](int x, int j, uint32_t (&w)[4]) {
#pragma unroll
      for (int c = 0; c < 4; ++c) w[c] = __ldg(p.v_sf + ((long long)x * p.tph_cap + j) * D + 32 * c + lane);
    };
    if constexpr (MX) {
      tmem_st_32x32b_x4(tmem + lane_addr + kSfP, kSfOne, kSfOne, kSfOne, kSfOne);
      tmem_st_wait();
    }
    int it = 0;
    for (int t = t_lo; t < t_hi;) {
      int x, j0, n, tn;
      next_segment(t, x, j0, n, tn);
      const int b = x / p.Hkv, h = x - b * p.Hkv;
      [[maybe_unused]] float q_scale_mine = 1.f;
      if constexpr (KV8 && !MX) {
        if (tid < D) { ch_scale[tid] = __ldg(p.kscale + (long long)x * D + tid); ch_scale[D + tid] = __ldg(p.vscale + (long long)x * D + tid); }
        named_bar_sync(1, kSmx);
      }
      {
        const int qr = tid >> 3, part8 = tid & 7;
        const bool qv = qr < R;
        const int g = qv ? qr / p.Sq : 0, qi = qv ? qr - g * p.Sq : 0;
        const uint16_t* src = reinterpret_cast<const uint16_t*>(p.q) + (long long)b * p.q_sb + (long long)(h * p.G + g) * p.q_sh +
                              (long long)qi * p.q_ss + part8 * 16;
        if constexpr (!KV8) {
          if (qv) {
#pragma unroll
            for (int u = 0; u < 2; ++u) {
              const int ch = part8 * 2 + u;
              const uint4 w = __ldg(reinterpret_cast<const uint4*>(src) + u);
              *reinterpret_cast<uint4*>(q_s + (ch >> 3) * SM::kQAtomBytes + qr * 128 + (((ch & 7) ^ (qr & 7)) << 4)) = w;
            }
          }
        } else if constexpr (MX) {
          float qf[16];
          float amax = 0.f;
#pragma unroll
          for (int u = 0; u < 16; ++u) {
            float v = 0.f;
// ... 127 lines not shown
          m4[4 * g4 + 2] = fmaxf(fmaxf(a0.z, a1.z), fmaxf(a2.z, a3.z));
          m4[4 * g4 + 3] = fmaxf(fmaxf(a0.w, a1.w), fmaxf(a2.w, a3.w));
        }
        float grow = sw_ninf();
#pragma unroll
        for (int qn = 0; qn < kSwN; ++qn) grow = fmaxf(grow, m4[qn] - m_used[qn]);
        if (grow > kSwRescale) {
          float alpha[kSwN];
#pragma unroll
          for (int qn = 0; qn < kSwN; ++qn) {
            const float m_new = fmaxf(m_used[qn], m4[qn]);
            alpha[qn] = (m_new == sw_ninf()) ? 1.f : fast_exp2(m_used[qn] - m_new);
            l_thr[qn] *= alpha[qn];
            m_used[qn] = m_new;
            neg_ms[qn] = (m_new == sw_ninf()) ? 0.f : -m_new;
          }
          if (jj > 0) {
            mbar_wait(&pv_done[(i - 1) & 1], ((i - 1) >> 1) & 1);
            tc_fence_after();
            uint32_t orow[16];
            tmem_ld_32x32b_x16(tmem_o + lane_addr, orow);
            tmem_ld_wait();
#pragma unroll
            for (int qn = 0; qn < kSwN; ++qn) orow[qn] = __float_as_uint(__uint_as_float(orow[qn]) * alpha[qn]);
            tmem_st_32x32b_x16(tmem_o + lane_addr, orow);
            tmem_st_wait();
          }
        }
        if (jj >= 2) { mbar_wait(&pv_done[i & 1], ((i - 2) >> 1) & 1); }
        const uint32_t pt = pt_a + uint32_t(i & 1) * SM::kPBytes;
#pragma unroll
        for (int qn = 0; qn < kSwN; ++qn) {
          const float pv = fast_exp2(sv[qn] + neg_ms[qn]);
          l_thr[qn] += pv;
          if constexpr (!KV8) {
            st_shared_u16(pt + pa[qn & 7] + qn * 128, sw_to16<BF16>(pv));
          } else {
            uint16_t e2;
            asm("cvt.rn.satfinite.e4m3x2.f32 %0, %1, %2;" : "=h"(e2) : "f"(0.f), "f"(pv));
            st_shared_u8(pt + pa[qn & 7] + qn * 128, e2);
          }
        }
        if constexpr (MX) {
          if (jj + 2 < n) tmem_st_32x32b_x4(tmem + lane_addr + kSfK + 4 * (i & 1), ksf_n[0], ksf_n[1], ksf_n[2], ksf_n[3]);
          tmem_st_32x32b_x4(tmem + lane_addr + kSfV + 4 * (i & 1), vsf_c[0], vsf_c[1], vsf_c[2], vsf_c[3]);
          tmem_st_wait();
        }
        fence_proxy_async_smem();
        tc_fence_before();
        __syncwarp();
        if (lane == 0) mbar_arrive(&p_full[i & 1]);
      }
      const dcomm::Tail tail = make_tail();
      int nparts, pidx;
      dcomm::head_parts(geo, x, cta, nparts, pidx);
      uint64_t* my_part = dcomm::part_ptr<D>(tail, x, pidx);
      {
        float lw[kSwN];
#pragma unroll
        for (int qn = 0; qn < kSwN; ++qn) {
          float v = l_thr[qn];
#pragma unroll
          for (int sft = 16; sft > 0; sft >>= 1) v += __shfl_xor_sync(0xffffffffu, v, sft);
          lw[qn] = v;
        }
        if (lane == 0) {
#pragma unroll
          for (int qn = 0; qn < kSwN; ++qn) red_s[warp * kSwN + qn] = lw[qn];
        }
        named_bar_sync(2, kSmx);
        uint32_t orow[16];
        if (n > 0) {
          const int il = it + n - 1;
          mbar_wait(&pv_done[il & 1], (il >> 1) & 1);
          tc_fence_after();
          tmem_ld_32x32b_x16(tmem_o + lane_addr, orow);
          tmem_ld_wait();
        } else {
#pragma unroll
          for (int qn = 0; qn < kSwN; ++qn) orow[qn] = 0u;
        }
        float vs_d = 1.f;
        if constexpr (KV8 && !MX) vs_d = ch_scale[D + row];
#pragma unroll
        for (int qn = 0; qn < kSwN; ++qn)
          if (qn < R) dcomm::ll_store_gpu(my_part + qn * (D + 2) + row, __uint_as_float(orow[qn]) * vs_d, tail.wtag);
        if (tid < R) {
          const float lsum = red_s[tid] + red_s[kSwN + tid] + red_s[2 * kSwN + tid] + red_s[3 * kSwN + tid];
          float mq = sw_ninf();
#pragma unroll
          for (int qn = 0; qn < kSwN; ++qn) mq = (qn == tid) ? m_used[qn] : mq;
          dcomm::ll_store_gpu(my_part + tid * (D + 2) + D, mq, tail.wtag);
          dcomm::ll_store_gpu(my_part + tid * (D + 2) + D + 1, lsum, tail.wtag);
        }
        tc_fence_before();
      }
      it += n;
      dcomm::segment_done<D, kSmx, 4>(tail, x, tn, n_pend, tid, 1, store_out);
      named_bar_sync(1, kSmx);
      t = tn;
    }
    const dcomm::Tail tail = make_tail();
    dcomm::drain<D, kSmx, 4>(tail, n_pend, tid, 1, store_out);
  }
  tc_fence_before();
  __syncthreads();
  if (warp == 5) { tc_fence_after(); tmem_dealloc<128>(tmem); }
}

// ... 64 lines not shown
```

### tree_attention_b200/csrc/decode_tc_sm100.cu

```cuda
#include "common.cuh"
#include "decode_comm.cuh"
#include "host_utils.h"
#include "kernels.h"

namespace ta {
namespace {

constexpr int kTM = 128;
constexpr int kTN = 128;
constexpr int kTcThreads = 192;
constexpr int kSmx = 128;
constexpr int kTcStages = 3;
constexpr int kTcMaxPending = 32;
constexpr float kTcRescale = 8.0f;

struct DecodeTcParams {
  const void* q;
  void* out;
  float* lse;
  uint64_t* part;
  unsigned long long* wctr;
  const float* kscale;
  const float* vscale;
  const int* kv_len;
// ... 11 lines not shown
  static constexpr int kElem = KV8 ? 1 : 2;
  static constexpr int kAtoms = D * kElem / 128;
  static constexpr int kTileBytes = 128 * D * kElem;
  static constexpr int kAtomBytes = 128 * 128;
  static constexpr int kStages = KV8 ? 6 : kTcStages;
  static constexpr size_t kTotal = 1024 + size_t(1 + 2 * kStages) * kTileBytes + 512 + (KV8 ? 2 * D * 4 : 0);
};

__device__ __forceinline__ float tc_ninf() { return __int_as_float(0xff800000); }
template <bool BF16>
__device__ __forceinline__ uint32_t tc_pack2(float lo, float hi) {
  if constexpr (BF16) return pack_bf16x2(lo, hi);
  else return pack_f16x2(lo, hi);
}
template <bool BF16>
__device__ __forceinline__ uint16_t tc_to16(float f) {
  if constexpr (BF16) return __bfloat16_as_ushort(__float2bfloat16_rn(f));
  else return __half_as_ushort(__float2half_rn(f));
}

template <int D, bool BF16, bool KV8>
__global__ void __launch_bounds__(kTcThreads, 1)
decode_tc_kernel(const __grid_constant__ CUtensorMap kmap, const __grid_constant__ CUtensorMap vmap,
                 const __grid_constant__ DecodeTcParams p) {
  using SM = TcSmem<D, KV8>;
  constexpr int NS = SM::kStages;
  constexpr int EPA = 128 / SM::kElem;
  extern __shared__ uint8_t smem_raw[];
  uint8_t* smem = reinterpret_cast<uint8_t*>((reinterpret_cast<uintptr_t>(smem_raw) + 1023) & ~uintptr_t(1023));
  uint8_t* q_s = smem;
  uint8_t* k_s = q_s + SM::kTileBytes;
  uint8_t* v_s = k_s + NS * SM::kTileBytes;
  uint64_t* bars = reinterpret_cast<uint64_t*>(v_s + NS * SM::kTileBytes);
  uint64_t* q_ready = bars;
  uint64_t* k_full = bars + 1;
  uint64_t* k_empty = k_full + NS;
  uint64_t* v_full = k_empty + NS;
  uint64_t* v_empty = v_full + NS;
  uint64_t* s_full = v_empty + NS;
  uint64_t* p_full = s_full + 2;
  uint64_t* pv_done = p_full + 2;
  uint64_t* stamps = pv_done + 2;
  uint32_t* tmem_slot = reinterpret_cast<uint32_t*>(stamps + 2);
  int* s_misc = reinterpret_cast<int*>(tmem_slot + 2);
  int* s_tags = s_misc + 4;
  int* pending = s_tags + 4;
  [[maybe_unused]] float* ch_scale = reinterpret_cast<float*>(pending + kTcMaxPending);

  const int tid = threadIdx.x, warp = tid >> 5, lane = tid & 31;
  const int cta = blockIdx.x;
  const int world = p.comm.world;
  const int BH = p.B * p.Hkv;
  const int R = p.R;
  const dcomm::Geom geo = dcomm::make_geom(p.S, p.kv_len, BH, gridDim.x);
  const int t_lo = dcomm::cta_lo(geo, cta), t_hi = dcomm::cta_lo(geo, cta + 1);
  int jvis = geo.tph;
  if (p.causal) {
    const long long last = p.q_pos0 + p.Sq - 1 - p.kv_pos0;
    jvis = (int)max(0LL, min((long long)geo.tph, last < 0 ? 0LL : last / kTN + 1));
  }
  const int n_active_warps = (R + 31) / 32;

  if (tid == 0) {
    mbar_init(q_ready, kSmx);
    for (int i = 0; i < NS; ++i) { mbar_init(&k_full[i], 1); mbar_init(&k_empty[i], 1); mbar_init(&v_full[i], 1); mbar_init(&v_empty[i], 1); }
    for (int i = 0; i < 2; ++i) { mbar_init(&s_full[i], 1); mbar_init(&p_full[i], n_active_warps); mbar_init(&pv_done[i], 1); }
    fence_mbar_init();
    s_misc[0] = 0; s_misc[1] = 0; s_tags[2] = 0;
  }
  if (warp == 4 && lane == 0) { tma_prefetch_desc(&kmap); tma_prefetch_desc(&vmap); }
  if (warp == 5) tmem_alloc<512>(tmem_slot);
  if (warp < 4) {
    for (int c = tid; c < SM::kTileBytes / 16; c += kSmx) reinterpret_cast<uint4*>(q_s)[c] = make_uint4(0, 0, 0, 0);
  }
  tc_fence_before();
  __syncthreads();
  tc_fence_after();
  const uint32_t tmem = *tmem_slot;
  const uint32_t tmem_o = tmem + 256;

  if (tid == 0) { stamps[0] = globaltimer_ns(); stamps[1] = 0; }

  auto next_segment = [&](int t, int& x, int& j0, int& n, int& t_next) {
    x = t / geo.tph;
    const int seg_end = min(t_hi, (x + 1) * geo.tph);
    j0 = t - x * geo.tph;
    const int j1 = seg_end - x * geo.tph;
    n = max(0, min(j1, jvis) - j0);
    t_next = seg_end;
  };

  if (warp == 4) {
    if (lane == 0) {
      int it = 0;
      bool tags_done = false;
      auto fetch_tags = [&]() {
        const uint32_t wtag = dcomm::launch_tag(p.wctr);
        const uint32_t ctag = world > 1 ? dcomm::launch_tag(reinterpret_cast<unsigned long long*>(p.comm.epoch)) : 0u;
        volatile int* sm = s_tags;
        sm[0] = (int)wtag; sm[1] = (int)ctag;
        __threadfence_block();
        sm[2] = 1;
        tags_done = true;
      };
      for (int t = t_lo; t < t_hi;) {
        int x, j0, n, tn;
        next_segment(t, x, j0, n, tn);
// ... 49 lines not shown
        next_segment(t, x, j0, n, tn);
        mbar_wait(q_ready, seg & 1);
        tc_fence_after();
        if (n > 0) {
          issue_qk(it);
          for (int jj = 0; jj < n; ++jj) {
            const int i = it + jj;
            if (jj + 1 < n) issue_qk(i + 1);
            const int st = i % NS;
            mbar_wait(&p_full[i & 1], (i >> 1) & 1);
            mbar_wait(&v_full[st], (i / NS) & 1);
            tc_fence_after();
            const uint64_t v_desc = umma_smem_desc_sw128(smem_u32(v_s + st * SM::kTileBytes), kTN * 128, 1024);
            const uint32_t p_tmem = tmem + (i & 1) * 128;
            if (leader) {
#pragma unroll
              for (int kk = 0; kk < kTN / KSTEP; ++kk) {
                if constexpr (KV8) umma_ts_f8(tmem_o, p_tmem + kk * 8, v_desc + ((kk * (KSTEP * 128)) >> 4), idesc_pv, (jj > 0 || kk > 0) ? 1u : 0u);
                else umma_ts_f16(tmem_o, p_tmem + kk * 8, v_desc + ((kk * (KSTEP * 128)) >> 4), idesc_pv, (jj > 0 || kk > 0) ? 1u : 0u);
              }
              umma_commit(&v_empty[st]);
              umma_commit(&pv_done[i & 1]);
            }
            __syncwarp();
          }
          it += n;
        }
        ++seg;
        t = tn;
      }
    }
    __syncwarp();
  } else {
    const int row = tid;
    const bool row_valid = row < R;
    const bool warp_active = (warp * 32) < R;
    const uint32_t lane_addr = uint32_t(warp * 32) << 16;
    const int g_row = row / p.Sq, i_row = row - g_row * p.Sq;
    const long long q_pos = p.q_pos0 + i_row;

    auto store_out = [&](int x, int r, int d, float o_norm, float lse2) {
      const int b = x / p.Hkv, h = x - b * p.Hkv;
      const int g = r / p.Sq, i = r - g * p.Sq;
      uint16_t* op = reinterpret_cast<uint16_t*>(p.out) + (long long)b * p.o_sb + (long long)(h * p.G + g) * p.o_sh +
                     (long long)i * p.o_ss + d;
      *op = tc_to16<BF16>(o_norm);
      if (d == 0 && p.lse != nullptr) p.lse[((long long)b * p.Hq + (h * p.G + g)) * p.Sq + i] = lse2 * 0.6931471805599453f;
    };
    int n_pend = 0;
    auto make_tail = [&]() {
      dcomm::Tail tl;
      volatile int* sm = s_tags;
      while (sm[2] == 0) { }
      tl.comm = &p.comm; tl.part = p.part; tl.max_parts = p.max_parts; tl.BH = BH;
      tl.R = R; tl.rows_valid = R; tl.wtag = (uint32_t)sm[0]; tl.ctag = (uint32_t)sm[1]; tl.geo = geo;
      tl.pending = pending; tl.max_pending = kTcMaxPending; tl.stamps = stamps;
      return tl;
    };

    int it = 0;
    for (int t = t_lo; t < t_hi;) {
      int x, j0, n, tn;
      next_segment(t, x, j0, n, tn);
      const int b = x / p.Hkv, h = x - b * p.Hkv;
      [[maybe_unused]] float q_scale = 1.f;
      if constexpr (KV8) {
        if (tid < D) {
          ch_scale[tid] = __ldg(p.kscale + (long long)x * D + tid);
          ch_scale[D + tid] = __ldg(p.vscale + (long long)x * D + tid);
        }
        named_bar_sync(1, kSmx);
      }
      if (row_valid) {
        const uint4* src = reinterpret_cast<const uint4*>(reinterpret_cast<const uint16_t*>(p.q) + (long long)b * p.q_sb +
                                                          (long long)(h * p.G + g_row) * p.q_sh + (long long)i_row * p.q_ss);
        if constexpr (!KV8) {
#pragma unroll
          for (int ch = 0; ch < D / 8; ++ch)
            *reinterpret_cast<uint4*>(q_s + (ch >> 3) * SM::kAtomBytes + row * 128 + (((ch & 7) ^ (row & 7)) << 4)) = __ldg(src + ch);
        } else {
          float qf[D];
          float amax = 0.f;
#pragma unroll
          for (int ch = 0; ch < D / 8; ++ch) {
            const uint4 w = __ldg(src + ch);
            const uint32_t ws[4] = {w.x, w.y, w.z, w.w};
#pragma unroll
            for (int u = 0; u < 4; ++u) {
              float lo, hi;
              if constexpr (BF16) { lo = bf16lo(ws[u]); hi = bf16hi(ws[u]); } else { lo = f16lo(ws[u]); hi = f16hi(ws[u]); }
              lo *= ch_scale[ch * 8 + 2 * u]; hi *= ch_scale[ch * 8 + 2 * u + 1];
              qf[ch * 8 + 2 * u] = lo; qf[ch * 8 + 2 * u + 1] = hi;
              amax = fmaxf(amax, fmaxf(fabsf(lo), fabsf(hi)));
            }
          }
          q_scale = amax > 0.f ? amax * (1.f / 448.f) : 1.f;
          const float inv = 1.f / q_scale;
#pragma unroll
          for (int ch = 0; ch < D / 16; ++ch) {
            uint4 w;
            w.x = pack_e4m3x4(qf[ch * 16 + 0] * inv, qf[ch * 16 + 1] * inv, qf[ch * 16 + 2] * inv, qf[ch * 16 + 3] * inv);
            w.y = pack_e4m3x4(qf[ch * 16 + 4] * inv, qf[ch * 16 + 5] * inv, qf[ch * 16 + 6] * inv, qf[ch * 16 + 7] * inv);
            w.z = pack_e4m3x4(qf[ch * 16 + 8] * inv, qf[ch * 16 + 9] * inv, qf[ch * 16 + 10] * inv, qf[ch * 16 + 11] * inv);
            w.w = pack_e4m3x4(qf[ch * 16 + 12] * inv, qf[ch * 16 + 13] * inv, qf[ch * 16 + 14] * inv, qf[ch * 16 + 15] * inv);
            *reinterpret_cast<uint4*>(q_s + row * 128 + (((ch & 7) ^ (row & 7)) << 4)) = w;
          }
        }
// ... 39 lines not shown
          if (__any_sync(0xffffffffu, refresh)) {
            const float alpha = refresh ? fast_exp2(m_used - m_new) : 1.f;
            if (refresh) { l_sum *= alpha; m_used = m_new; }
            if (jj > 0) {
              mbar_wait(&pv_done[(i - 1) & 1], ((i - 1) >> 1) & 1);
              tc_fence_after();
#pragma unroll
              for (int c0 = 0; c0 < D; c0 += 32) {
                uint32_t orow[32];
                tmem_ld_32x32b_x32(tmem_o + lane_addr + c0, orow);
                tmem_ld_wait();
#pragma unroll
                for (int u = 0; u < 32; ++u) orow[u] = __float_as_uint(__uint_as_float(orow[u]) * alpha);
                tmem_st_32x32b_x32(tmem_o + lane_addr + c0, orow);
              }
            }
          }
          const float neg_m = (m_used == tc_ninf()) ? 0.f : -m_used;
          float ls[8] = {0.f, 0.f, 0.f, 0.f, 0.f, 0.f, 0.f, 0.f};
          if constexpr (!KV8) {
            uint32_t pk[64];
#pragma unroll
            for (int c = 0; c < 128; c += 8) {
#pragma unroll
              for (int u = 0; u < 8; u += 2) {
                const float p0 = fast_exp2(fmaf(__uint_as_float(sr[c + u]), sc_row, neg_m));
                const float p1 = fast_exp2(fmaf(__uint_as_float(sr[c + u + 1]), sc_row, neg_m));
                ls[u] += p0; ls[u + 1] += p1;
                pk[(c + u) >> 1] = tc_pack2<BF16>(p0, p1);
              }
            }
            tmem_st_32x32b_x32(s_tmem + 0, *reinterpret_cast<uint32_t(*)[32]>(&pk[0]));
            tmem_st_32x32b_x32(s_tmem + 32, *reinterpret_cast<uint32_t(*)[32]>(&pk[32]));
          } else {
            uint32_t pk[32];
#pragma unroll
            for (int c = 0; c < 128; c += 8) {
              float pv[8];
#pragma unroll
              for (int u = 0; u < 8; ++u) { pv[u] = fast_exp2(fmaf(__uint_as_float(sr[c + u]), sc_row, neg_m)); ls[u] += pv[u]; }
              pk[c >> 2] = pack_e4m3x4(pv[0], pv[1], pv[2], pv[3]);
              pk[(c >> 2) + 1] = pack_e4m3x4(pv[4], pv[5], pv[6], pv[7]);
            }
            tmem_st_32x32b_x32(s_tmem, pk);
          }
          l_sum += ((ls[0] + ls[1]) + (ls[2] + ls[3])) + ((ls[4] + ls[5]) + (ls[6] + ls[7]));
          tmem_st_wait();
          tc_fence_before();
          __syncwarp();
          if (lane == 0) mbar_arrive(&p_full[i & 1]);
        }
      }
      const dcomm::Tail tail = make_tail();
      int nparts, pidx;
      dcomm::head_parts(geo, x, cta, nparts, pidx);
      uint64_t* my_part = dcomm::part_ptr<D>(tail, x, pidx);
      if (warp_active) {
        if (n > 0) {
          const int il = it + n - 1;
          mbar_wait(&pv_done[il & 1], (il >> 1) & 1);
          tc_fence_after();
        }
#pragma unroll
        for (int c0 = 0; c0 < D; c0 += 32) {
          uint32_t orow[32];
          if (n > 0) {
            tmem_ld_32x32b_x32(tmem_o + lane_addr + c0, orow);
            tmem_ld_wait();
          } else {
#pragma unroll
            for (int u = 0; u < 32; ++u) orow[u] = 0u;
          }
          if (row_valid) {
            uint64_t* dst = my_part + row * (D + 2) + c0;
#pragma unroll
            for (int u = 0; u < 32; ++u) {
              float o1 = __uint_as_float(orow[u]);
              if constexpr (KV8) o1 *= ch_scale[D + c0 + u];
              dcomm::ll_store_gpu(dst + u, o1, tail.wtag);
            }
          }
        }
        if (row_valid) {
          dcomm::ll_store_gpu(my_part + row * (D + 2) + D, m_used, tail.wtag);
          dcomm::ll_store_gpu(my_part + row * (D + 2) + D + 1, l_sum, tail.wtag);
        }
        tc_fence_before();
      }
      it += n;
      dcomm::segment_done<D, kSmx, 4>(tail, x, tn, n_pend, tid, 1, store_out);
      named_bar_sync(1, kSmx);
      t = tn;
    }
    const dcomm::Tail tail = make_tail();
    dcomm::drain<D, kSmx, 4>(tail, n_pend, tid, 1, store_out);
  }
  tc_fence_before();
  __syncthreads();
  if (warp == 5) { tc_fence_after(); tmem_dealloc<512>(tmem); }
}

template <int D, bool BF16, bool KV8>
std::function<void(cudaStream_t)> make_tc_pass(const CUtensorMap& kmap, const CUtensorMap& vmap, const DecodeTcParams& p, int grid) {
  auto kern = decode_tc_kernel<D, BF16, KV8>;
  static bool configured = false;
  if (!configured) {
    TA_CUDA_CHECK(cudaFuncSetAttribute(kern, cudaFuncAttributeMaxDynamicSharedMemorySize, (int)TcSmem<D, KV8>::kTotal));
    configured = true;
  }
// ... 70 lines not shown
```

### tree_attention_b200/csrc/kernels.h

```cpp
#pragma once
#include <cuda_runtime.h>
#include <stdint.h>

#include <functional>
#include <vector>

namespace ta {

struct PreparedLaunch {
  std::vector<std::function<void(cudaStream_t)>> passes;
  void run(cudaStream_t stream) const {
    for (const auto& f : passes) f(stream);
  }
};

constexpr int kMaxWorldHost = 16;

struct CommCtxHost {
  int rank = 0;
  int world = 1;
  void* data[kMaxWorldHost] = {nullptr};
  void* flags[kMaxWorldHost] = {nullptr};
  void* epoch = nullptr;
  void* status = nullptr;
  unsigned long long timeout_ns = 10ull * 1000 * 1000 * 1000;
  int skip_publish = 0;
  size_t data_bytes = 0;
  size_t flag_bytes = 0;
};

struct AttnShape {
  int B = 1, Hq = 1, Hkv = 1, Sq = 1, S = 0, D = 128;
  int is_bf16 = 1;
  float softmax_scale = 1.f;
  int causal = 0;
  int64_t q_pos0 = 0;
  int64_t kv_pos0 = 0;
  int kv_seg_len = 0;
  int64_t kv_seg_gap = 0;
  int64_t q_sb = 0, q_sh = 0, q_ss = 0;
  int64_t k_sb = 0, k_sh = 0, k_ss = 0;
  int64_t v_sb = 0, v_sh = 0, v_ss = 0;
  int64_t o_sb = 0, o_sh = 0, o_ss = 0;
};

void decode_split(int BH, int cap, int ncta, int* grid, int* max_parts);

void decode_simt_plan(const AttnShape& s, int num_sms, int* grid, int* max_parts, int* rows_per_pass,
                      size_t* part_floats, size_t* comm_floats, size_t* comm_flags);
void decode_simt_launch(const AttnShape& s, const void* q, const void* k, const void* v, void* out, float* lse,
                        float* part, uint32_t* tickets, const CommCtxHost& comm, int num_sms,
                        cudaStream_t stream, const uint32_t* kscale = nullptr, const uint32_t* vscale = nullptr,
                        int pdl = 0, const int* kv_len = nullptr);
void decode_simt_set_trace(unsigned long long* buf);
PreparedLaunch decode_simt_prepare(const AttnShape& s, const void* q, const void* k, const void* v, void* out, float* lse,
                                   float* part, uint32_t* tickets, const CommCtxHost& comm, int num_sms,
                                   const uint32_t* kscale = nullptr, const uint32_t* vscale = nullptr, int pdl = 0,
                                   const int* kv_len = nullptr);

void decode_tc_split(const AttnShape& s, int ncta, int* grid, int* max_parts);
void decode_tc_plan(const AttnShape& s, int num_sms, int* grid, int* max_parts, int* rows, size_t* part_floats,
                    size_t* comm_bytes);
void decode_tc_launch(const AttnShape& s, const void* q, const void* k, const void* v, void* out, float* lse, float* part,
                      uint32_t* tickets, const CommCtxHost& comm, int num_sms, cudaStream_t stream,
                      const float* kscale = nullptr, const float* vscale = nullptr, const int* kv_len = nullptr);
PreparedLaunch decode_tc_prepare(const AttnShape& s, const void* q, const void* k, const void* v, void* out, float* lse,
                                 float* part, uint32_t* tickets, const CommCtxHost& comm, int num_sms,
                                 const float* kscale = nullptr, const float* vscale = nullptr,
                                 const int* kv_len = nullptr);

void decode_swap_launch(const AttnShape& s, const void* q, const void* k, const void* v, void* out, float* lse, float* part,
                        uint32_t* tickets, const CommCtxHost& comm, int num_sms, cudaStream_t stream,
                        const float* kscale = nullptr, const float* vscale = nullptr, const uint32_t* k_sf = nullptr,
                        const uint32_t* v_sf = nullptr, const int* kv_len = nullptr);
PreparedLaunch decode_swap_prepare(const AttnShape& s, const void* q, const void* k, const void* v, void* out, float* lse,
                                   float* part, uint32_t* tickets, const CommCtxHost& comm, int num_sms,
                                   const float* kscale = nullptr, const float* vscale = nullptr,
                                   const uint32_t* k_sf = nullptr, const uint32_t* v_sf = nullptr,
                                   const int* kv_len = nullptr);

void combine_launch(const float* o_part, const float* lse_part, void* out, int out_dtype, float* lse_out,
                    int64_t rows, int D, const CommCtxHost& comm, int mode, cudaStream_t stream);

void umma_probe_launch(const void* a, const void* b, float* c, int N, int K, int b_mn_major, int a_from_tmem,
                       cudaStream_t stream);

long long tmem_ld_bw_probe(int warps, int iters, cudaStream_t stream);
void umma_2cta_probe_launch(const void* a, const void* b, float* c, int N, cudaStream_t stream);
void umma_bs_probe_launch(const void* a8, const void* b8, const void* sfa, const void* sfb, float* c, int N,
                          cudaStream_t stream, int a_mn_major = 0);

void attn_fwd_launch(const AttnShape& s, const void* q, const void* k, const void* v, void* out, float* lse,
                     const CommCtxHost& comm, cudaStream_t stream, int q_in_tmem = 0, int comm_mode = 1, int sq_out = 0);
void attn_fwd_phase_cycles(unsigned long long* out5);
size_t attn_fwd_comm_bytes(const AttnShape& s, int world, size_t* flag_bytes, int comm_mode = 1);
void attn_bwd_launch(const AttnShape& s, const void* q, const void* k, const void* v, const void* o, const void* dout,
                     const float* lse, float* dq, void* dk, void* dv, float* delta, float* lse2, int64_t do_sb,
                     int64_t do_sh, int64_t do_ss, cudaStream_t stream);

// ... 13 lines not shown
```

### tree_attention_b200/ops/local.py

```python
from __future__ import annotations

from typing import Dict, Optional, Tuple

import torch

from .. import _build
from . import reference as ref

_WS: Dict[tuple, Dict[str, torch.Tensor]] = {}

DECODE_MAX_ROWS = 128


def _as_bhsd(x: torch.Tensor) -> torch.Tensor:
    if x.stride(-1) != 1:
        x = x.contiguous()
    return x


def new_workspace(device: torch.device, nfloats: int, nticket: int) -> Dict[str, torch.Tensor]:
    return {
        "part": torch.zeros(max(nfloats, 2), dtype=torch.float32, device=device),
        "tickets": torch.zeros(max(nticket, 64), dtype=torch.int32, device=device),
    }
# ... 15 lines not shown
        if kv_len.dtype != torch.int32 or kv_len.device != like.device:
            kv_len = kv_len.to(device=like.device, dtype=torch.int32)
        return kv_len.reshape(1)
    return torch.tensor([int(kv_len)], dtype=torch.int32, device=like.device)


def decode_eligible(q: torch.Tensor, k: torch.Tensor) -> bool:
    if not q.is_cuda or q.dtype not in (torch.bfloat16, torch.float16):
        return False
    d = q.shape[-1]
    g = q.shape[1] // k.shape[1]
    return d in (64, 128) and q.shape[2] * g <= DECODE_MAX_ROWS


def decode_attention(
    q: torch.Tensor,
    k: torch.Tensor,
    v: torch.Tensor,
    softmax_scale: float,
    causal: bool = False,
    q_pos0: int = 0,
    kv_pos0: int = 0,
    comm=None,
    out: Optional[torch.Tensor] = None,
    lse: Optional[torch.Tensor] = None,
    return_lse: bool = True,
    impl: str = "auto",
    pdl: int = 0,
    kv_len=None,
) -> Tuple[torch.Tensor, Optional[torch.Tensor]]:
    import os

    C = _build.load()
    q, k, v = _as_bhsd(q), _as_bhsd(k), _as_bhsd(v)
    b, hq, sq, d = q.shape
    hkv, s = k.shape[1], k.shape[2]
    rows_total = (hq // hkv) * sq
    impl = os.environ.get("TREE_ATTN_DECODE_IMPL", impl)
    if impl == "auto":
        impl = "simt" if rows_total == 1 else ("swap" if (rows_total <= 16 and d == 128) else "tc")
    if impl in ("tc", "swap"):
        if q.stride(2) % 8 != 0 and sq > 1:
            q = q.contiguous()
        grid, max_parts, rows, part_floats, _ = C.decode_tc_plan(b, hq, hkv, sq, s, d)
        ws = _workspace(q.device, "decode_tc", part_floats, b * hkv + 2)
        if out is None:
            out = torch.empty((b, hq, sq, d), dtype=q.dtype, device=q.device)
        if lse is None and return_lse:
            lse = torch.empty((b, hq, sq), dtype=torch.float32, device=q.device)
        C.decode_tc_fwd(q, k, v, out, lse, ws["part"], ws["tickets"], comm, float(softmax_scale), bool(causal),
                        int(q_pos0), int(kv_pos0), impl == "swap", _kv_len_arg(kv_len, k))
        return out, lse
    grid, max_parts, rows, part_floats, _, _ = C.decode_plan(b, hq, hkv, sq, s, d)
    ws = _workspace(q.device, "decode", part_floats, b * hkv + 2)
    if out is None:
        out = torch.empty((b, hq, sq, d), dtype=q.dtype, device=q.device)
    if lse is None and return_lse:
        lse = torch.empty((b, hq, sq), dtype=torch.float32, device=q.device)
    C.decode_fwd(q, k, v, out, lse, ws["part"], ws["tickets"], comm, float(softmax_scale), bool(causal),
                 int(q_pos0), int(kv_pos0), int(os.environ.get("TREE_ATTN_PDL", pdl)), _kv_len_arg(kv_len, k))
    return out, lse


def decode_impl_for(q_shape, k_shape, impl: str = "auto") -> str:
    import os

    b, hq, sq, d = q_shape
    rows_total = (hq // k_shape[1]) * sq
    impl = os.environ.get("TREE_ATTN_DECODE_IMPL", impl)
    if impl == "auto":
        impl = "simt" if rows_total == 1 else ("swap" if (rows_total <= 16 and d == 128) else "tc")
    return impl


def decode_workspace_sizes(q_shape, k_shape, impl: str) -> Tuple[int, int]:
    C = _build.load()
    b, hq, sq, d = q_shape
    hkv, s = k_shape[1], k_shape[2]
    if impl in ("tc", "swap"):
        part_floats = C.decode_tc_plan(b, hq, hkv, sq, s, d)[3]
    else:
        part_floats = C.decode_plan(b, hq, hkv, sq, s, d)[3]
    return int(part_floats), b * hkv + 2


def decode_attention_mxfp8(
    q: torch.Tensor,
    k,
    v,
    softmax_scale: float,
    causal: bool = False,
    q_pos0: int = 0,
    kv_pos0: int = 0,
    comm=None,
    return_lse: bool = True,
    kv_len=None,
) -> Tuple[torch.Tensor, Optional[torch.Tensor]]:
    C = _build.load()
    q = _as_bhsd(q)
    b, hq, sq, d = q.shape
    hkv, s = k.shape[1], k.shape[2]
    grid, max_parts, rows, part_floats, _, _ = C.decode_plan(b, hq, hkv, sq, s, d)
    ws = _workspace(q.device, "decode", part_floats, b * hkv + 2)
    out = torch.empty((b, hq, sq, d), dtype=q.dtype, device=q.device)
    lse = torch.empty((b, hq, sq), dtype=torch.float32, device=q.device) if return_lse else None
    C.decode_fwd_mx(q, k.data, v.data, k.scales, v.scales, out, lse, ws["part"], ws["tickets"], comm,
                    float(softmax_scale), bool(causal), int(q_pos0), int(kv_pos0), _kv_len_arg(kv_len, k.data))
    return out, lse


def decode_attention_fp8(
    q: torch.Tensor,
    k,
    v,
    softmax_scale: float,
    causal: bool = False,
    q_pos0: int = 0,
    kv_pos0: int = 0,
    comm=None,
    return_lse: bool = True,
    impl: str = "auto",
    kv_len=None,
) -> Tuple[torch.Tensor, Optional[torch.Tensor]]:
    C = _build.load()
    q = _as_bhsd(q)
    b, hq, sq, d = q.shape
    hkv, s = k.shape[1], k.shape[2]
    if q.stride(2) % 8 != 0 and sq > 1:
        q = q.contiguous()
    grid, max_parts, rows, part_floats, _ = C.decode_tc_plan(b, hq, hkv, sq, s, d)
    ws = _workspace(q.device, "decode_tc", part_floats, b * hkv + 2)
    out = torch.empty((b, hq, sq, d), dtype=q.dtype, device=q.device)
    lse = torch.empty((b, hq, sq), dtype=torch.float32, device=q.device) if return_lse else None
    import os

    impl = os.environ.get("TREE_ATTN_DECODE_FP8_IMPL", impl)
    if impl == "auto":
        impl = "swap" if rows <= 16 else "tc"
    C.decode_tc_fwd8(q, k.data, v.data, k.scales, v.scales, out, lse, ws["part"], ws["tickets"], comm,
                     float(softmax_scale), bool(causal), int(q_pos0), int(kv_pos0), impl == "swap", _kv_len_arg(kv_len, k.data))
    return out, lse


def decode_attention_mx_tc(
    q: torch.Tensor,
    k,
    v,
    softmax_scale: float,
    causal: bool = False,
    q_pos0: int = 0,
    kv_pos0: int = 0,
    comm=None,
    return_lse: bool = True,
    kv_len=None,
) -> Tuple[torch.Tensor, Optional[torch.Tensor]]:
    C = _build.load()
# ... 71 lines not shown
```

Baseline: 407.5 million.

## Add tail work-stealing pool to SIMT decode split with chunked partial slots

```diff
diff --git a/bench_tools/hbm_read_ceiling.py b/bench_tools/hbm_read_ceiling.py
--- /dev/null
+++ b/bench_tools/hbm_read_ceiling.py
@@ -0,0 +1,89 @@
+import argparse
+import json
+import os
+import subprocess
+import tempfile
+
+import torch
+from torch.utils.cpp_extension import load_inline
+
+CUDA_SRC = r"""
+#include <torch/extension.h>
+#include <ATen/cuda/CUDAContext.h>
+
+__global__ void read_stream(const uint4* __restrict__ src, long long n16, unsigned* sink) {
+  uint4 acc = make_uint4(0, 0, 0, 0);
+  const long long stride = (long long)gridDim.x * blockDim.x;
+  long long i = (long long)blockIdx.x * blockDim.x + threadIdx.x;
+  for (; i + 3 * stride < n16; i += 4 * stride) {
+    uint4 w[4];
+#pragma unroll
+    for (int u = 0; u < 4; ++u)
+      asm volatile("ld.global.nc.L1::no_allocate.v4.u32 {%0,%1,%2,%3}, [%4];"
+                   : "=r"(w[u].x), "=r"(w[u].y), "=r"(w[u].z), "=r"(w[u].w) : "l"(src + i + u * stride));
+#pragma unroll
+    for (int u = 0; u < 4; ++u) { acc.x ^= w[u].x; acc.y ^= w[u].y; acc.z ^= w[u].z; acc.w ^= w[u].w; }
+  }
+  for (; i < n16; i += stride) { const uint4 w = src[i]; acc.x ^= w.x; acc.y ^= w.y; acc.z ^= w.z; acc.w ^= w.w; }
+  if ((acc.x ^ acc.y ^ acc.z ^ acc.w) == 0x9e3779b9u) sink[0] = 1;   // practically never true: keeps the loads alive
+}
+
+void read_stream_launch(torch::Tensor buf, torch::Tensor sink, int64_t ctas, int64_t threads) {
+  read_stream<<<(int)ctas, (int)threads, 0, at::cuda::getCurrentCUDAStream()>>>(
+      reinterpret_cast<const uint4*>(buf.data_ptr()), buf.numel() * buf.element_size() / 16,
+      reinterpret_cast<unsigned*>(sink.data_ptr()));
+}
+"""
+CPP_SRC = "void read_stream_launch(torch::Tensor buf, torch::Tensor sink, int64_t ctas, int64_t threads);"
+
+
+def main():
+    ap = argparse.ArgumentParser()
+    ap.add_argument("--seq", type=int, default=131072)
+    ap.add_argument("--heads", type=int, default=32)
+    ap.add_argument("--dim", type=int, default=128)
+    ap.add_argument("--ctas-per-sm", type=int, nargs="*", default=[1, 2, 4, 8])
+    ap.add_argument("--threads", type=int, default=512)
+    ap.add_argument("--reps", type=int, default=50)
+    a = ap.parse_args()
+    build_dir = tempfile.mkdtemp(prefix="hbm_read_ceiling_")
+    mod = load_inline("hbm_read_ceiling", cpp_sources=CPP_SRC, cuda_sources=CUDA_SRC, functions=["read_stream_launch"],
+                      extra_cuda_cflags=["-O3", "-gencode", "arch=compute_100a,code=sm_100a"], build_directory=build_dir)
+    dev = torch.device("cuda")
+    nbytes = 2 * a.seq * a.heads * a.dim * 2
+    nbuf = max(2, -(-4 * (126 << 20) // nbytes) + 1)
+    bufs = [torch.randint(0, 1 << 30, (nbytes // 4,), dtype=torch.int32, device=dev) for _ in range(nbuf)]
+    sink = torch.zeros(1, dtype=torch.int32, device=dev)
+    nsm = torch.cuda.get_device_properties(dev).multi_processor_count
+    res = {"bytes_per_step": nbytes, "buffers_rotated": nbuf}
+    try:
+        q = subprocess.run(["nvidia-smi", "--query-gpu=name,power.limit,clocks.max.sm", "--format=csv,noheader"],
+                           capture_output=True, text=True, timeout=20).stdout.strip()
+        res["gpu"] = q.splitlines()[torch.cuda.current_device()] if q else None
+    except Exception:
+        res["gpu"] = None
+    best = None
+    for cps in a.ctas_per_sm:
+        ctas = nsm * cps
+        for i in range(2 * nbuf):
+            mod.read_stream_launch(bufs[i % nbuf], sink, ctas, a.threads)
+        torch.cuda.synchronize()
+        e0, e1 = torch.cuda.Event(enable_timing=True), torch.cuda.Event(enable_timing=True)
+        e0.record()
+        for i in range(a.reps):
+            mod.read_stream_launch(bufs[i % nbuf], sink, ctas, a.threads)
+        e1.record()
+        torch.cuda.synchronize()
+        us = e0.elapsed_time(e1) / a.reps * 1e3
+        tbps = nbytes / us / 1e6
+        res[f"ctas_per_sm_{cps}"] = {"us_per_pass": round(us, 2), "read_TBps": round(tbps, 3)}
+        if best is None or us < best[0]:
+            best = (us, tbps, cps)
+    res["best_us_per_pass"] = round(best[0], 2)
+    res["best_read_TBps"] = round(best[1], 3)
+    res["best_ctas_per_sm"] = best[2]
+    print(json.dumps(res), flush=True)
+
+
+if __name__ == "__main__":
+    main()
diff --git a/bench_tools/trace_decode.py b/bench_tools/trace_decode.py
--- a/bench_tools/trace_decode.py
+++ b/bench_tools/trace_decode.py
@@ -77,20 +77,12 @@
         res["producer_issue_span_us"] = stat(us(t[:, 11] - t[:, 10]))
         per_tile = us(t[:, 5] - t[:, 4]) / (t[:, 12] - 1).clamp(min=1)
         res["us_per_tile"] = stat(per_tile)
-        sw = t[t[:, 14] > 0]
-        if len(sw):
-            fin = (sw[:, 14].long() & 0xffffffff).double()
-            ldq = (sw[:, 14].long() >> 32).double()
-            wt = (sw[:, 15].long() & 0xffffffff).double()
-            pos = (sw[:, 15].long() >> 32).double()
-            res["switch_finalize_us"] = stat(us(fin))
-            res["switch_load_q_us"] = stat(us(ldq))
-            res["switch_wait_next_tile_us"] = stat(us(wt))
-            res["switch_tile_index"] = stat(pos)
-            before = us(sw[:, 7] - sw[:, 4]) / pos.clamp(min=1)
-            after = us(sw[:, 5] - sw[:, 7]) / (sw[:, 12] - pos).clamp(min=1)
-            res["switch_cta_us_per_tile_before"] = stat(before)
-            res["switch_cta_us_per_tile_after"] = stat(after)
+        res["pieces_per_cta"] = stat(t[:, 14])
+        res["stolen_per_cta"] = stat(t[:, 15])
+        res["pieces_total"] = int(t[:, 14].sum())
+        end = us(t[:, 5] - t[:, 1]) + (t[:, 0] - g0) / 1e3
+        res["stream_end_us_after_first_entry(min,med,max)"] = stat(end)
+        res["stream_end_spread_us"] = round(float(end.max() - end.min()), 2)
         if os.environ.get("TRACE_DUMP"):
             torch.save(t, os.path.join(os.environ["TRACE_DUMP"], f"trace_{S}.pt"))
         print(json.dumps(res), flush=True)
diff --git a/tree_attention_b200/csrc/bindings.cpp b/tree_attention_b200/csrc/bindings.cpp
--- a/tree_attention_b200/csrc/bindings.cpp
+++ b/tree_attention_b200/csrc/bindings.cpp
@@ -5,6 +5,7 @@
 
 #include <cstring>
 
+#include "decode_geom.h"
 #include "host_utils.h"
 #include "kernels.h"
 
@@ -114,7 +115,7 @@
   c10::cuda::CUDAGuard guard(q.device());
   AttnShape s = make_shape(q, k, v, out, scale, causal, q_pos0, kv_pos0);
   TORCH_CHECK(part.scalar_type() == at::kFloat && part.is_contiguous(), "part must be contiguous fp32");
-  TORCH_CHECK(tickets.scalar_type() == at::kInt && tickets.numel() >= s.B * s.Hkv + 2, "tickets too small");
+  TORCH_CHECK(tickets.scalar_type() == at::kInt && tickets.numel() >= std::max(s.B * s.Hkv + 2, ta::decode_simt_ticket_ints()), "tickets too small");
   int grid, mp, R;
   size_t pf, cf, cfl;
   ta::decode_simt_plan(s, ta::num_sms(), &grid, &mp, &R, &pf, &cf, &cfl);
@@ -306,7 +307,7 @@
   int grid, mp, R;
   size_t pf, cf, cfl;
   ta::decode_simt_plan(s, ta::num_sms(), &grid, &mp, &R, &pf, &cf, &cfl);
-  TORCH_CHECK((size_t)part.numel() >= pf && tickets.numel() >= s.B * s.Hkv + 2, "workspace too small");
+  TORCH_CHECK((size_t)part.numel() >= pf && tickets.numel() >= std::max(s.B * s.Hkv + 2, ta::decode_simt_ticket_ints()), "workspace too small");
   float* lse_p = lse.has_value() ? lse->data_ptr<float>() : nullptr;
   CommCtxHost c;
   if (!comm.is_none()) c = comm.cast<Comm&>().h;
@@ -371,6 +372,7 @@
     size_t pf, cf, cfl;
     ta::decode_simt_plan(s, ta::num_sms(), &grid, &mp, &R, &pf, &cf, &cfl);
     TORCH_CHECK((size_t)part.numel() >= pf, "part workspace too small: need ", pf, " floats");
+    TORCH_CHECK(tickets.numel() >= ta::decode_simt_ticket_ints(), "tickets too small");
     for (int pdl = 0; pdl < 3; ++pdl) {
       st->launches[pdl] = ta::decode_simt_prepare(s, io_ptr(q), k.data_ptr(), v.data_ptr(), io_ptr(out), lse_p,
                                                   part.data_ptr<float>(), tk, c, ta::num_sms(), nullptr, nullptr, pdl, kvl);
@@ -594,6 +596,32 @@
     ta::umma_2cta_probe_launch(a.data_ptr(), b.data_ptr(), c.data_ptr<float>(), 128, at::cuda::getCurrentCUDAStream());
   });
   m.def("num_sms", []() { return ta::num_sms(); });
+  m.def("decode_ticket_ints", &ta::decode_simt_ticket_ints);
+  m.def("decode_steal_geom", [](int B, int Hkv, int cap, int s, int ncta) {
+    int g = 0, mp = 0;
+    ta::decode_split(B * Hkv, cap, ncta, &g, &mp);
+    const ta::dcomm::Geom geo = ta::dcomm::geom_for(std::max(0, std::min(cap, s)), B * Hkv, g, true);
+    std::vector<std::tuple<int, int, int, int>> ranges;
+    for (int c = 0; c < g; ++c)
+      ranges.emplace_back(ta::dcomm::cta_lo(geo, c), ta::dcomm::pool_lo(geo, c), ta::dcomm::cta_lo(geo, c + 1),
+                          ta::dcomm::num_chunks(geo, c));
+    std::vector<int> slots;
+    for (int x = 0; x < B * Hkv; ++x) slots.push_back(ta::dcomm::head_slots(geo, x));
+    return py::make_tuple(g, ta::decode_simt_max_slots(mp), geo.chunk, ranges, slots);
+  });
+  m.def("decode_steal_chunk", [](int B, int Hkv, int cap, int s, int ncta, int c, int k) {
+    int g = 0, mp = 0;
+    ta::decode_split(B * Hkv, cap, ncta, &g, &mp);
+    const ta::dcomm::Geom geo = ta::dcomm::geom_for(std::max(0, std::min(cap, s)), B * Hkv, g, true);
+    int b = 0, e = 0;
+    ta::dcomm::chunk_tiles(geo, c, k, b, e);
+    return py::make_tuple(b, e, ta::dcomm::seg_slot(geo, b / geo.tph, b));
+  });
+  m.def("decode_steal_slot", [](int B, int Hkv, int cap, int s, int ncta, int x, int t) {
+    int g = 0, mp = 0;
+    ta::decode_split(B * Hkv, cap, ncta, &g, &mp);
+    return ta::dcomm::seg_slot(ta::dcomm::geom_for(std::max(0, std::min(cap, s)), B * Hkv, g, true), x, t);
+  });
   m.def("decode_split_for", [](int B, int Hkv, int S, int ncta) {
     AttnShape s{};
     s.B = B; s.Hkv = Hkv; s.Hq = Hkv; s.Sq = 1; s.S = S; s.D = 128;
diff --git a/tree_attention_b200/csrc/common.cuh b/tree_attention_b200/csrc/common.cuh
--- a/tree_attention_b200/csrc/common.cuh
+++ b/tree_attention_b200/csrc/common.cuh
@@ -138,6 +138,9 @@
 __device__ __forceinline__ void mbar_arrive_expect_tx(uint64_t* bar, uint32_t bytes) {
   asm volatile("mbarrier.arrive.expect_tx.shared::cta.b64 _, [%0], %1;" ::"r"(smem_u32(bar)), "r"(bytes)
                : "memory");
+}
+__device__ __forceinline__ void mbar_expect_tx(uint64_t* bar, uint32_t bytes) {
+  asm volatile("mbarrier.expect_tx.relaxed.cta.shared::cta.b64 [%0], %1;" ::"r"(smem_u32(bar)), "r"(bytes) : "memory");
 }
 __device__ __forceinline__ bool mbar_try_wait(uint64_t* bar, uint32_t parity) {
   uint32_t ok;
diff --git a/tree_attention_b200/csrc/decode_comm.cuh b/tree_attention_b200/csrc/decode_comm.cuh
--- a/tree_attention_b200/csrc/decode_comm.cuh
+++ b/tree_attention_b200/csrc/decode_comm.cuh
@@ -1,37 +1,19 @@
 #pragma once
 #include "common.cuh"
+#include "decode_geom.h"
 #include "kernels.h"
 
 namespace ta {
 namespace dcomm {
 
-constexpr int kTileKeys = 128;
-constexpr int kPartChunk = 8;
+constexpr int kPartChunk = 16;
 
 __device__ __forceinline__ float ninf() { return __int_as_float(0xff800000); }
 
-struct Geom {
-  int S;
-  int tph;
-  int total;
-  int tiles_q, tiles_rem;
-};
-
-__device__ __forceinline__ Geom make_geom(int cap, const int* kv_len, int BH, int ncta) {
-  Geom g;
+__device__ __forceinline__ Geom make_geom(int cap, const int* kv_len, int BH, int ncta, bool steal) {
   int s = cap;
   if (kv_len != nullptr) s = max(0, min(cap, *reinterpret_cast<const volatile int*>(kv_len)));
-  g.S = s;
-  g.tph = max(1, (s + kTileKeys - 1) / kTileKeys);
-  g.total = BH * g.tph;
-  g.tiles_q = g.total / ncta;
-  g.tiles_rem = g.total - g.tiles_q * ncta;
-  return g;
-}
-__device__ __forceinline__ int cta_lo(const Geom& g, int c) { return c * g.tiles_q + min(c, g.tiles_rem); }
-__device__ __forceinline__ int cta_of_tile(const Geom& g, int t) {
-  const int big = g.tiles_rem * (g.tiles_q + 1);
-  return t < big ? t / (g.tiles_q + 1) : g.tiles_rem + (t - big) / max(g.tiles_q, 1);
+  return geom_for(s, BH, ncta, steal);
 }
 
 __device__ __forceinline__ void ll_store_sys(uint64_t* w, float v, uint32_t tag) {
@@ -66,19 +48,10 @@
   }
   return out;
 }
-static __device__ __noinline__ uint64_t ll_spin_gpu(const uint64_t* w, uint32_t tag) {
-  const uint64_t t0 = globaltimer_ns();
-  uint32_t it = 0;
-  uint64_t out;
-  while (true) {
-    out = ll_load_gpu(w);
-    if (ll_tag(out) == tag) break;
-    if ((++it & 0x3fu) == 0 && globaltimer_ns() - t0 > TA_SPIN_TIMEOUT_NS) {
-      printf("[tree_attention] split-merge wait timeout block=%d thread=%d tag=%u\n", blockIdx.x, threadIdx.x, tag);
-      __trap();
-    }
-  }
-  return out;
+
+static __device__ __noinline__ void merge_wait_timeout(int x, uint32_t tag) {
+  printf("[tree_attention] split-merge wait timeout block=%d thread=%d head=%d tag=%u\n", blockIdx.x, threadIdx.x, x, tag);
+  __trap();
 }
 
 constexpr int kTagShift = 12;
@@ -92,7 +65,7 @@
 struct Tail {
   const CommCtx* comm;
   uint64_t* part;
-  int max_parts;
+  int max_slots;
   int BH;
   int R;
   int rows_valid;
@@ -106,19 +79,13 @@
 
 template <int D>
 __device__ __forceinline__ uint64_t* part_ptr(const Tail& t, int x, int pidx) {
-  return t.part + ((size_t)x * t.max_parts + pidx) * (size_t)(t.R * (D + 2));
+  return t.part + ((size_t)x * t.max_slots + pidx) * (size_t)(t.R * (D + 2));
 }
 template <int D>
 __device__ __forceinline__ uint64_t* word_ptr(const Tail& t, int dst, int src, int x) {
   return reinterpret_cast<uint64_t*>(t.comm->data[dst]) +
          ((size_t)((t.ctag & 1) * t.comm->world + src) * t.BH + x) * (size_t)(t.R * (D + 2));
 }
-__device__ __forceinline__ void head_parts(const Geom& g, int x, int cta, int& nparts, int& pidx) {
-  const int first_cta = cta_of_tile(g, x * g.tph);
-  nparts = cta_of_tile(g, (x + 1) * g.tph - 1) - first_cta + 1;
-  pidx = cta - first_cta;
-}
-
 template <int D>
 __device__ __forceinline__ void merge_parts(const Tail& t, int x, int nparts, int r, int d, float& o_norm, float& lse2) {
   const size_t pstride = (size_t)t.R * (D + 2);
@@ -126,12 +93,22 @@
   float M = ninf(), acc = 0.f, L = 0.f;
   for (int q0 = 0; q0 < nparts; q0 += kPartChunk) {
     uint64_t wa[kPartChunk], wm[kPartChunk], wl[kPartChunk];
-#pragma unroll
-    for (int i = 0; i < kPartChunk; ++i) {
-      if (q0 + i < nparts) {
-        const uint64_t* pp = base + (size_t)(q0 + i) * pstride;
-        wa[i] = ll_load_gpu(pp + d); wm[i] = ll_load_gpu(pp + D); wl[i] = ll_load_gpu(pp + D + 1);
-      }
+    uint64_t t0 = 0;
+    for (uint32_t it = 0;; ++it) {
+      bool ready = true;
+#pragma unroll
+      for (int i = 0; i < kPartChunk; ++i) {
+        if (q0 + i < nparts) {
+          const uint64_t* pp = base + (size_t)(q0 + i) * pstride;
+          wa[i] = ll_load_gpu(pp + d); wm[i] = ll_load_gpu(pp + D); wl[i] = ll_load_gpu(pp + D + 1);
+        }
+      }
+#pragma unroll
+      for (int i = 0; i < kPartChunk; ++i)
+        if (q0 + i < nparts) ready &= ll_tag(wa[i]) == t.wtag && ll_tag(wm[i]) == t.wtag && ll_tag(wl[i]) == t.wtag;
+      if (ready) break;
+      if (it == 0) t0 = globaltimer_ns();
+      else if ((it & 0x3fu) == 0 && globaltimer_ns() - t0 > TA_SPIN_TIMEOUT_NS) merge_wait_timeout(x, t.wtag);
     }
     float m[kPartChunk], a[kPartChunk], l[kPartChunk];
     float Mn = M;
@@ -139,10 +116,6 @@
     for (int i = 0; i < kPartChunk; ++i) {
       m[i] = ninf(); a[i] = 0.f; l[i] = 0.f;
       if (q0 + i < nparts) {
-        const uint64_t* pp = base + (size_t)(q0 + i) * pstride;
-        if (ll_tag(wa[i]) != t.wtag) wa[i] = ll_spin_gpu(pp + d, t.wtag);
-        if (ll_tag(wm[i]) != t.wtag) wm[i] = ll_spin_gpu(pp + D, t.wtag);
-        if (ll_tag(wl[i]) != t.wtag) wl[i] = ll_spin_gpu(pp + D + 1, t.wtag);
         a[i] = ll_val(wa[i]); m[i] = ll_val(wm[i]); l[i] = ll_val(wl[i]);
         Mn = fmaxf(Mn, m[i]);
       }
@@ -273,8 +246,7 @@
 __device__ __noinline__ void merge_head(const Tail& t, int x, int tid, StoreOut& store_out) {
   static_assert(NT % D == 0, "thread count must be a multiple of head_dim");
   constexpr int NG = NT / D;
-  int nparts, pidx;
-  head_parts(t.geo, x, blockIdx.x, nparts, pidx);
+  const int nparts = head_slots(t.geo, x);
   const int world = t.comm->world;
   const int d = tid % D;
   for (int r = tid / D; r < t.rows_valid; r += NG) {
diff --git a/tree_attention_b200/csrc/decode_geom.h b/tree_attention_b200/csrc/decode_geom.h
--- /dev/null
+++ b/tree_attention_b200/csrc/decode_geom.h
@@ -0,0 +1,92 @@
+#pragma once
+
+#if defined(__CUDACC__)
+#define TA_HD __host__ __device__ __forceinline__
+#else
+#define TA_HD inline
+#endif
+
+namespace ta {
+namespace dcomm {
+
+constexpr int kTileKeys = 128;
+constexpr int kStealTailPct = 20;
+constexpr int kStealChunks = 8;
+constexpr int kSlotsPerRange = kStealChunks + 2;
+constexpr int kStealCounters = 1024;
+constexpr int kDecodeTicketInts = 2 + 2 * 2 * kStealCounters;
+
+TA_HD int gmin(int a, int b) { return a < b ? a : b; }
+TA_HD int gmax(int a, int b) { return a > b ? a : b; }
+
+struct Geom {
+  int S;
+  int tph;
+  int total;
+  int tiles_q, tiles_rem;
+  int tail_pct;
+  int chunk;
+  int cph;
+};
+
+TA_HD Geom geom_for(int s, int BH, int ncta, bool steal) {
+  Geom g;
+  g.S = s;
+  g.tph = gmax(1, (s + kTileKeys - 1) / kTileKeys);
+  g.total = BH * g.tph;
+  g.tiles_q = g.total / ncta;
+  g.tiles_rem = g.total - g.tiles_q * ncta;
+  g.tail_pct = steal ? kStealTailPct : 0;
+  const int tail_max = (g.tiles_q + (g.tiles_rem > 0)) * g.tail_pct / 100;
+  g.chunk = gmax(1, (tail_max + kStealChunks - 1) / kStealChunks);
+  g.cph = (g.tph + g.chunk - 1) / g.chunk;
+  return g;
+}
+
+TA_HD int cta_lo(const Geom& g, int c) { return c * g.tiles_q + gmin(c, g.tiles_rem); }
+TA_HD int cta_of_tile(const Geom& g, int t) {
+  const int big = g.tiles_rem * (g.tiles_q + 1);
+  return t < big ? t / (g.tiles_q + 1) : g.tiles_rem + (t - big) / gmax(g.tiles_q, 1);
+}
+TA_HD int pool_lo(const Geom& g, int c) {
+  const int lo = cta_lo(g, c), hi = cta_lo(g, c + 1);
+  return hi - (hi - lo) * g.tail_pct / 100;
+}
+TA_HD int cuts_below(const Geom& g, int t) {
+  const int x = t / g.tph, j = t - x * g.tph;
+  return x * g.cph + (j + g.chunk - 1) / g.chunk;
+}
+TA_HD int cut_at(const Geom& g, int n) { return (n / g.cph) * g.tph + (n % g.cph) * g.chunk; }
+
+TA_HD int num_chunks(const Geom& g, int c) {
+  const int a = pool_lo(g, c), hi = cta_lo(g, c + 1);
+  return a < hi ? 1 + cuts_below(g, hi) - cuts_below(g, a + 1) : 0;
+}
+TA_HD void chunk_tiles(const Geom& g, int c, int k, int& s, int& e) {
+  const int a = pool_lo(g, c), hi = cta_lo(g, c + 1);
+  const int base = cuts_below(g, a + 1), n = 1 + cuts_below(g, hi) - base;
+  s = k == 0 ? a : cut_at(g, base + k - 1);
+  e = k + 1 == n ? hi : cut_at(g, base + k);
+}
+
+TA_HD int range_piece_starts(const Geom& g, int c, int xs, int t) {
+  const int lo = cta_lo(g, c), hi = cta_lo(g, c + 1), a = pool_lo(g, c);
+  int n = 0;
+  if (lo > xs && lo <= t) ++n;
+  if (a > lo && a < hi && a > xs && a <= t) ++n;
+  const int u0 = gmax(a, xs) + 1, u1 = gmin(hi - 1, t) + 1;
+  if (u1 > u0) n += cuts_below(g, u1) - cuts_below(g, u0);
+  return n;
+}
+TA_HD int seg_slot(const Geom& g, int x, int t) {
+  const int xs = x * g.tph;
+  const int c0 = cta_of_tile(g, xs), c1 = cta_of_tile(g, t);
+  if (g.tail_pct == 0) return c1 - c0;
+  int n = 0;
+  for (int c = c0; c <= c1; ++c) n += range_piece_starts(g, c, xs, t);
+  return n;
+}
+TA_HD int head_slots(const Geom& g, int x) { return seg_slot(g, x, (x + 1) * g.tph - 1) + 1; }
+
+}
+}
diff --git a/tree_attention_b200/csrc/decode_simt.cu b/tree_attention_b200/csrc/decode_simt.cu
--- a/tree_attention_b200/csrc/decode_simt.cu
+++ b/tree_attention_b200/csrc/decode_simt.cu
@@ -30,7 +30,7 @@
   int causal;
   long long q_pos0, kv_pos0;
   long long q_sb, q_sh, q_ss, o_sb, o_sh, o_ss;
-  int max_parts;
+  int max_slots;
   unsigned long long* trace;
   int pdl;
   CommCtx comm;
@@ -44,14 +44,21 @@
   static constexpr int kStageBytes = 2 * kTensorBytes;
   static constexpr int kStages = (D * kElem == 256) ? 3 : 6;
   static constexpr int kPsPerWarp = KV8 ? 4 : 1;
+  static constexpr int kQElem = KV8 ? 2 : 4;
 };
+
+struct StageDesc {
+  int x, j, slot, flags;
+};
+constexpr int kDescFirst = 1;
+constexpr int kDescNewQ = 2;
 
 template <int D, int R, bool KV8>
 constexpr size_t smem_bytes() {
   using L = SmemLayout<D, KV8>;
-  return 1024  + size_t(L::kStages) * L::kStageBytes +
-         sizeof(float) * (2 * R * D + kConsumerWarps * L::kPsPerWarp * R * kRowsPerWarp +
-                          (R <= 2 ? 2 : 1) * kConsumerWarps * R * (D + 4)) +
+  return 1024  + size_t(L::kStages) * (L::kStageBytes + sizeof(StageDesc) + R * D * 2) +
+         2 * R * D * L::kQElem +
+         sizeof(float) * (kConsumerWarps * L::kPsPerWarp * R * kRowsPerWarp + (R <= 2 ? 2 : 1) * kConsumerWarps * R * (D + 4)) +
          sizeof(int) * (kMaxPending + 8) + sizeof(uint64_t) * (2 * L::kStages + 2);
 }
 
@@ -88,11 +95,14 @@
   extern __shared__ uint8_t smem_raw[];
   uint8_t* smem = reinterpret_cast<uint8_t*>((reinterpret_cast<uintptr_t>(smem_raw) + 1023) & ~uintptr_t(1023));
   uint8_t* stage_base = smem;
-  float* q_s = reinterpret_cast<float*>(smem + size_t(NS) * L::kStageBytes);
-  float* p_s = q_s + 2 * R * D;
+  StageDesc* desc_s = reinterpret_cast<StageDesc*>(smem + size_t(NS) * L::kStageBytes);
+  float* q_s = reinterpret_cast<float*>(desc_s + NS);
+  constexpr int kQBuf = R * D * L::kQElem / 4;
+  float* p_s = q_s + 2 * kQBuf;
   float* merge_s = p_s + kConsumerWarps * L::kPsPerWarp * R * kRowsPerWarp;
   constexpr int kMergeBufs = R <= 2 ? 2 : 1;
-  int* pending = reinterpret_cast<int*>(merge_s + kMergeBufs * kConsumerWarps * R * (D + 4));
+  uint16_t* qraw_s = reinterpret_cast<uint16_t*>(merge_s + kMergeBufs * kConsumerWarps * R * (D + 4));
+  int* pending = reinterpret_cast<int*>(qraw_s + NS * R * D);
   int* s_misc = pending + kMaxPending;
   uint64_t* full_bar = reinterpret_cast<uint64_t*>(s_misc + 8);
   uint64_t* empty_bar = full_bar + NS;
@@ -108,7 +118,7 @@
     trc[0] = globaltimer_ns(); trc[1] = clock64();
     uint32_t smid;
     asm volatile("mov.u32 %0, %%smid;" : "=r"(smid));
-    trc[13] = smid; trc[14] = 0; trc[15] = 0;
+    trc[13] = smid;
   }
 
   if (tid == 0) {
@@ -117,7 +127,7 @@
       mbar_init(&empty_bar[i], kConsumerWarps);
     }
     fence_mbar_init();
-    s_misc[0] = 0; s_misc[1] = 0; s_misc[6] = 0;
+    s_misc[6] = 0;
   }
   if (warp == kConsumerWarps && lane == 0) {
     tma_prefetch_desc(&kmap);
@@ -135,50 +145,158 @@
   };
 
   if (warp == kConsumerWarps) {
-    if (lane == 0) {
-      if (p.pdl == 1) asm volatile("griddepcontrol.wait;" ::: "memory");
-      const dcomm::Geom geo = dcomm::make_geom(p.S, p.kv_len, BH, gridDim.x);
-      const int t_lo = dcomm::cta_lo(geo, cta), t_hi = dcomm::cta_lo(geo, cta + 1);
-      int stage = 0, issued = 0;
-      uint32_t phase = 0;
-      bool tags_done = false;
-      auto fetch_tags = [&]() {
-        if (p.pdl == 2) asm volatile("griddepcontrol.wait;" ::: "memory");
-        const uint32_t wtag = dcomm::launch_tag(p.wctr);
-        const uint32_t ctag = world > 1 ? dcomm::launch_tag(reinterpret_cast<unsigned long long*>(p.comm.epoch)) : 0u;
+    if (p.pdl == 1) asm volatile("griddepcontrol.wait;" ::: "memory");
+    const dcomm::Geom geo = dcomm::make_geom(p.S, p.kv_len, BH, gridDim.x, !KV8);
+    const int t_lo = dcomm::cta_lo(geo, cta), t_pool = dcomm::pool_lo(geo, cta);
+    unsigned long long* ctrs = p.wctr + 1;
+    int stage = 0, emitted = 0, committed = 0, loaded = 0, prev_x = -1;
+    uint32_t phase = 0, wtag = 0;
+    int pieces = 0, stolen = 0;
+    bool tags_done = false;
+    auto commit = [&](int st) {
+      const StageDesc dsc = desc_s[st];
+      if (dsc.x >= 0 && (dsc.flags & kDescNewQ)) {
+        const int b = dsc.x / p.Hkv, h = dsc.x - b * p.Hkv;
+        uint16_t* qd = qraw_s + st * R * D;
+        uint16_t val[R * D / 32];
+#pragma unroll
+        for (int u = 0; u < R * D / 32; ++u) {
+          const int idx = lane + 32 * u;
+          const int r = idx / D, d = idx - r * D;
+          val[u] = 0;
+          if (r < p.rows_valid) {
+            const int rr = p.r_base + r;
+            const int g = rr / p.Sq, i = rr - g * p.Sq;
+            val[u] = reinterpret_cast<const uint16_t*>(p.q)[(long long)b * p.q_sb + (long long)(h * p.G + g) * p.q_sh +
+                                                            (long long)i * p.q_ss + d];
+          }
+        }
+#pragma unroll
+        for (int u = 0; u < R * D / 32; ++u) qd[lane + 32 * u] = val[u];
+      }
+      __syncwarp();
+      if (lane == 0) mbar_arrive(&full_bar[st]);
+    };
+    auto fetch_tags = [&]() {
+      if (p.pdl == 2) asm volatile("griddepcontrol.wait;" ::: "memory");
+      uint32_t ctag = 0;
+      if (lane == 0) {
+        wtag = dcomm::launch_tag(p.wctr);
+        ctag = world > 1 ? dcomm::launch_tag(reinterpret_cast<unsigned long long*>(p.comm.epoch)) : 0u;
+      }
+      wtag = __shfl_sync(0xffffffffu, wtag, 0);
+      unsigned long long* other = ctrs + (size_t)((wtag & 1) ^ 1) * dcomm::kStealCounters;
+      for (int c = cta + lane * (int)gridDim.x; c < dcomm::kStealCounters; c += 32 * (int)gridDim.x) other[c] = 0ull;
+      if (lane == 0) {
         volatile int* sm = s_misc;
         sm[4] = (int)wtag; sm[5] = (int)ctag;
         __threadfence_block();
         sm[6] = 1;
-        tags_done = true;
-      };
-      for (int t = t_lo; t < t_hi; ++t) {
+      }
+      tags_done = true;
+      for (; committed < emitted; ++committed) commit(committed);
+    };
+    auto emit = [&](int x, int j, int slot, bool first) {
+      if (emitted == NS && !tags_done) fetch_tags();
+      if (lane == 0) mbar_wait(&empty_bar[stage], phase ^ 1);
+      __syncwarp();
+      const bool load = x >= 0 && tile_visible(j);
+      if (lane == 0) {
+        StageDesc dsc;
+        dsc.x = x; dsc.j = j; dsc.slot = slot; dsc.flags = (first ? kDescFirst : 0) | (x != prev_x ? kDescNewQ : 0);
+        desc_s[stage] = dsc;
+        if (load) {
+          if (trc && loaded == 0) trc[10] = clock64();
+          const int b = x / p.Hkv, h = x - b * p.Hkv;
+          mbar_expect_tx(&full_bar[stage], L::kStageBytes);
+          uint8_t* ks = stage_base + size_t(stage) * L::kStageBytes;
+          uint8_t* vs = ks + L::kTensorBytes;
+#pragma unroll
+          for (int a = 0; a < L::kAtoms; ++a) {
+            tma_load_4d(ks + a * (kTileRows * 128), &kmap, &full_bar[stage], a * (128 / L::kElem), j * kTileRows, h, b);
+            tma_load_4d(vs + a * (kTileRows * 128), &vmap, &full_bar[stage], a * (128 / L::kElem), j * kTileRows, h, b);
+          }
+        }
+      }
+      __syncwarp();
+      if (x >= 0) prev_x = x;
+      loaded += load;
+      ++emitted;
+      if (tags_done || p.pdl != 2) {
+        commit(stage);
+        ++committed;
+      }
+      if (++stage == NS) { stage = 0; phase ^= 1; }
+    };
+    auto warp_seg_slot = [&](int x, int t) {
+      const int xs = x * geo.tph;
+      const int c0 = dcomm::cta_of_tile(geo, xs), c1 = dcomm::cta_of_tile(geo, t);
+      if (geo.tail_pct == 0) return c1 - c0;
+      int n = 0;
+      for (int c = c0 + lane; c <= c1; c += 32) n += dcomm::range_piece_starts(geo, c, xs, t);
+      return (int)__reduce_add_sync(0xffffffffu, (unsigned)n);
+    };
+    auto run_piece = [&](int s, int e) {
+      for (int t = s; t < e; ++t) {
         const int x = t / geo.tph, j = t - x * geo.tph;
-        if (!tile_visible(j)) continue;
-        const int b = x / p.Hkv, h = x - b * p.Hkv;
-        if (issued == NS && !tags_done) fetch_tags();
-        mbar_wait(&empty_bar[stage], phase ^ 1);
-        if (trc && issued == 0) trc[10] = clock64();
-        mbar_arrive_expect_tx(&full_bar[stage], L::kStageBytes);
-        uint8_t* ks = stage_base + size_t(stage) * L::kStageBytes;
-        uint8_t* vs = ks + L::kTensorBytes;
-#pragma unroll
-        for (int a = 0; a < L::kAtoms; ++a) {
-          tma_load_4d(ks + a * (kTileRows * 128), &kmap, &full_bar[stage], a * (128 / L::kElem), j * kTileRows, h, b);
-          tma_load_4d(vs + a * (kTileRows * 128), &vmap, &full_bar[stage], a * (128 / L::kElem), j * kTileRows, h, b);
-        }
-        ++issued;
-        if (++stage == NS) { stage = 0; phase ^= 1; }
-      }
+        const bool first = t == s || j == 0;
+        if (!first && !tile_visible(j)) continue;
+        emit(x, j, first ? warp_seg_slot(x, t) : 0, first);
+      }
+      ++pieces;
+    };
+    if (t_lo < t_pool) run_piece(t_lo, t_pool);
+    if (geo.tail_pct > 0) {
       if (!tags_done) fetch_tags();
-      if (trc) { trc[11] = clock64(); trc[12] = (unsigned long long)issued; }
-    }
+      unsigned long long* ctr = ctrs + (size_t)(wtag & 1) * dcomm::kStealCounters;
+      const int n_own = dcomm::num_chunks(geo, cta);
+      unsigned long long nxt = 0;
+      if (lane == 0 && n_own > 0) nxt = atomicAdd(ctr + cta, 1ull);
+      for (int got = 0; got < n_own;) {
+        const unsigned long long old = __shfl_sync(0xffffffffu, nxt, 0);
+        const int lo = (int)(uint32_t)old, hi = (int)(old >> 32);
+        if (lo + hi >= n_own) break;
+        ++got;
+        if (lane == 0 && got < n_own) nxt = atomicAdd(ctr + cta, 1ull);
+        int s, e;
+        dcomm::chunk_tiles(geo, cta, lo, s, e);
+        run_piece(s, e);
+        if (got == n_own) break;
+      }
+      while (true) {
+        int best = 0, victim = 0;
+        for (int c = lane; c < (int)gridDim.x; c += 32) {
+          const uint64_t v = dcomm::ll_load_gpu(reinterpret_cast<const uint64_t*>(ctr + c));
+          const int left = dcomm::num_chunks(geo, c) - (int)(uint32_t)v - (int)(v >> 32);
+          if (left > best) { best = left; victim = c; }
+        }
+#pragma unroll
+        for (int o = 16; o > 0; o >>= 1) {
+          const int ob = __shfl_xor_sync(0xffffffffu, best, o), ov = __shfl_xor_sync(0xffffffffu, victim, o);
+          if (ob > best || (ob == best && ov < victim)) { best = ob; victim = ov; }
+        }
+        if (best <= 0) break;
+        unsigned long long old = 0;
+        if (lane == 0) old = atomicAdd(ctr + victim, 1ull << 32);
+        old = __shfl_sync(0xffffffffu, old, 0);
+        const int lo = (int)(uint32_t)old, hi = (int)(old >> 32), n = dcomm::num_chunks(geo, victim);
+        if (lo + hi >= n) continue;
+        int s, e;
+        dcomm::chunk_tiles(geo, victim, n - 1 - hi, s, e);
+        run_piece(s, e);
+        ++stolen;
+      }
+    }
+    if (trc && lane == 0) trc[11] = clock64();
+    emit(-1, 0, 0, false);
+    if (!tags_done) fetch_tags();
+    if (trc && lane == 0) { trc[12] = (unsigned long long)loaded; trc[14] = pieces; trc[15] = stolen; }
     return;
   }
 
   if (p.pdl) asm volatile("griddepcontrol.wait;" ::: "memory");
   if (trc && tid == 0) trc[3] = clock64();
-  const dcomm::Geom geo = dcomm::make_geom(p.S, p.kv_len, BH, gridDim.x);
+  const dcomm::Geom geo = dcomm::make_geom(p.S, p.kv_len, BH, gridDim.x, !KV8);
   const int t_lo = dcomm::cta_lo(geo, cta), t_hi = dcomm::cta_lo(geo, cta + 1);
   constexpr int RB = R;
   if (tid == 0) { stamps[0] = globaltimer_ns(); stamps[1] = 0; }
@@ -186,7 +304,7 @@
     dcomm::Tail tl;
     volatile int* sm = s_misc;
     while (sm[6] == 0) { }
-    tl.comm = &p.comm; tl.part = p.part; tl.max_parts = p.max_parts; tl.BH = BH;
+    tl.comm = &p.comm; tl.part = p.part; tl.max_slots = p.max_slots; tl.BH = BH;
     tl.R = R; tl.rows_valid = p.rows_valid; tl.wtag = (uint32_t)sm[4]; tl.ctag = (uint32_t)sm[5]; tl.geo = geo;
     tl.pending = pending; tl.max_pending = kMaxPending; tl.stamps = stamps;
     return tl;
@@ -194,7 +312,7 @@
   const int r16 = lane & 15;
   const int half = lane >> 4;
   float m_run[R], l_run[R], o_acc[R][EPL];
-  int cur_x = -1;
+  int cur_x = -1, cur_slot = 0;
   int stage = 0;
   uint32_t phase = 0;
 
@@ -208,32 +326,17 @@
     }
   };
 
-  auto load_q = [&](int x, int buf) {
-    const int b = x / p.Hkv, h = x - b * p.Hkv;
+  auto load_q = [&](const uint16_t* src, int buf) {
     for (int idx = tid; idx < R * D; idx += kConsumerThreads) {
-      const int r = idx / D, d = idx - r * D;
-      float val = 0.f;
-      if (r < p.rows_valid) {
-        const int rr = p.r_base + r;
-        const int g = rr / p.Sq, i = rr - g * p.Sq;
-        const uint16_t* qp = reinterpret_cast<const uint16_t*>(p.q) + (long long)b * p.q_sb +
-                             (long long)(h * p.G + g) * p.q_sh + (long long)i * p.q_ss + d;
-        val = cvt1<BF16>(*qp) * p.scale_log2;
-      }
-      if constexpr (KV8) reinterpret_cast<__half*>(q_s + buf * R * D)[idx] = __float2half_rn(val);
-      else q_s[buf * R * D + idx] = val;
+      const float val = cvt1<BF16>(src[idx]) * p.scale_log2;
+      if constexpr (KV8) reinterpret_cast<__half*>(q_s + buf * kQBuf)[idx] = __float2half_rn(val);
+      else q_s[buf * kQBuf + idx] = val;
     }
   };
-  const int x_first = t_lo / geo.tph;
-  if (t_lo < t_hi) {
-    load_q(x_first, 0);
-    if ((x_first + 1) * geo.tph < t_hi) load_q(x_first + 1, 1);
-  }
-  named_bar_sync(1, kConsumerThreads);
   const float* q_cur = q_s;
+  int q_next = 0;
   uint32_t wtag = 0;
   int n_fin = 0;
-  int n_pend = 0;
 
   auto store_out = [&](int x, int r, int d, float o_norm, float lse2) {
     const int b = x / p.Hkv, h = x - b * p.Hkv;
@@ -246,7 +349,7 @@
       p.lse[((long long)b * p.Hq + (h * p.G + g)) * p.Sq + i] = lse2 * 0.6931471805599453f;
   };
 
-  auto finalize_segment = [&](int x) {
+  auto finalize_segment = [&](int x, int slot, const uint16_t* qsrc) {
     float* mbuf = merge_s + (kMergeBufs == 2 ? (n_fin & 1) : 0) * (kConsumerWarps * R * (D + 4));
     ++n_fin;
 #pragma unroll
@@ -261,15 +364,14 @@
       for (int e = 0; e < EPL; ++e) ms[lane * EPL + e] = o_acc[r][e];
       if (lane == 0) { ms[D] = m_run[r]; ms[D + 1] = lt; }
     }
+    if (qsrc != nullptr) load_q(qsrc, q_next);
     named_bar_sync(1, kConsumerThreads);
     if (wtag == 0) {
       volatile int* sm = s_misc;
       while (sm[6] == 0) { }
       wtag = (uint32_t)sm[4];
     }
-    int nparts, pidx;
-    dcomm::head_parts(geo, x, cta, nparts, pidx);
-    uint64_t* my_part = p.part + ((size_t)x * p.max_parts + pidx) * (size_t)(R * (D + 2));
+    uint64_t* my_part = p.part + ((size_t)x * p.max_slots + slot) * (size_t)(R * (D + 2));
     for (int idx = tid; idx < R * D; idx += kConsumerThreads) {
       const int r = idx / D, d = idx - r * D;
       float M = neg_inf();
@@ -289,10 +391,6 @@
         dcomm::ll_store_gpu(my_part + r * (D + 2) + D, M, wtag);
         dcomm::ll_store_gpu(my_part + r * (D + 2) + D + 1, Lsum, wtag);
       }
-    }
-    if (min(t_hi, (x + 1) * geo.tph) == (x + 1) * geo.tph) {
-      if (tid == 0) pending[n_pend] = x;
-      ++n_pend;
     }
     if constexpr (kMergeBufs == 1) named_bar_sync(1, kConsumerThreads);
   };
@@ -332,35 +430,31 @@
       v_sw[k7] = uint32_t(L::kTensorBytes + atom * (kTileRows * 128) + off + ((chunk ^ k7) << 4) + (warp * kRowsPerWarp) * 128);
   }
 
-  for (int t = t_lo; t < t_hi; ++t) {
-    const int x = t / geo.tph, j = t - x * geo.tph;
+  for (int n_tiles = 0;; ++n_tiles) {
+    mbar_wait(&full_bar[stage], phase);
+    const StageDesc dsc = desc_s[stage];
+    if (dsc.x < 0) break;
+    const int x = dsc.x, j = dsc.j;
     [[maybe_unused]] const uint32_t ksc_word = nxt_ksc;
     [[maybe_unused]] const uint32_t vsc_cur = nxt_vsc;
-    fetch_scales(t + 1);
-    bool switched = false;
-    long long ts0 = 0, ts1 = 0, ts2 = 0;
-    if (x != cur_x) {
-      switched = cur_x >= 0;
-      ts0 = clock64();
-      if (cur_x >= 0) finalize_segment(cur_x);
-      ts1 = clock64();
-      const int rel = x - x_first;
-      if (rel >= 2) {
-        load_q(x, rel & 1);
+    fetch_scales(tile_visible(j + 1) ? x * geo.tph + j + 1 : (x + 1) * geo.tph);
+    if (trc && tid == 0 && n_tiles == 0) trc[4] = clock64();
+    if (dsc.flags & kDescFirst) {
+      const uint16_t* qsrc = (dsc.flags & kDescNewQ) ? qraw_s + stage * R * D : nullptr;
+      if (cur_x >= 0) {
+        finalize_segment(cur_x, cur_slot, qsrc);
+      } else if (qsrc != nullptr) {
+        load_q(qsrc, q_next);
         named_bar_sync(1, kConsumerThreads);
       }
-      q_cur = q_s + (rel & 1) * R * D;
+      if (qsrc != nullptr) { q_cur = q_s + q_next * kQBuf; q_next ^= 1; }
       reset_state();
-      cur_x = x;
-      ts2 = clock64();
-    }
-    if (!tile_visible(j)) continue;
-    mbar_wait(&full_bar[stage], phase);
-    if (trc && tid == 0 && t == t_lo) trc[4] = clock64();
-    if (trc && tid == 0 && switched) {
-      trc[14] = (unsigned long long)(ts1 - ts0) | ((unsigned long long)(ts2 - ts1) << 32);
-      trc[15] = (unsigned long long)(clock64() - ts2) | ((unsigned long long)(t - t_lo) << 32);
-      trc[7] = (unsigned long long)ts0;
+      cur_x = x; cur_slot = dsc.slot;
+    }
+    if (!tile_visible(j)) {
+      if (lane == 0) mbar_arrive(&empty_bar[stage]);
+      if (++stage == NS) { stage = 0; phase ^= 1; }
+      continue;
     }
     const uint8_t* ks = stage_base + size_t(stage) * L::kStageBytes;
     const uint8_t* vs = ks + L::kTensorBytes;
@@ -547,9 +641,13 @@
     if (++stage == NS) { stage = 0; phase ^= 1; }
   }
   if (trc && tid == 0) trc[5] = clock64();
-  if (cur_x >= 0) finalize_segment(cur_x);
+  if (cur_x >= 0) finalize_segment(cur_x, cur_slot, nullptr);
   if (trc && tid == 0) trc[6] = clock64();
 
+  const int x_merge0 = t_lo / geo.tph;
+  const int n_pend = max(0, t_hi / geo.tph - x_merge0);
+  if (tid == 0)
+    for (int i = 0; i < n_pend; ++i) pending[i] = x_merge0 + i;
   const dcomm::Tail tail = make_tail();
   dcomm::drain<D, kConsumerThreads, RB>(tail, n_pend, tid, 1, store_out);
   if (trc && tid == 0) { trc[8] = clock64(); trc[9] = globaltimer_ns(); }
@@ -587,6 +685,9 @@
 
 void decode_simt_set_trace(unsigned long long* buf) { g_decode_trace = buf; }
 
+int decode_simt_max_slots(int max_parts) { return max_parts * dcomm::kSlotsPerRange; }
+int decode_simt_ticket_ints() { return dcomm::kDecodeTicketInts; }
+
 void decode_split(int BH, int cap, int ncta, int* grid, int* max_parts) {
   const int tph = std::max(1, (cap + kTileRows - 1) / kTileRows);
   const long long total = (long long)BH * tph;
@@ -602,7 +703,7 @@
   decode_split(BH, s.S, nsm, grid, max_parts);
   const int R = pick_rows((s.Hq / s.Hkv) * s.Sq);
   *rows_per_pass = R;
-  *part_floats = (size_t)BH * *max_parts * R * (s.D + 2) * 2;
+  *part_floats = (size_t)BH * decode_simt_max_slots(*max_parts) * R * (s.D + 2) * 2;
   *comm_floats = (size_t)2 * kMaxWorldHost * BH * R * (s.D + 2) * 2;
   *comm_flags = (size_t)2 * kMaxWorldHost * BH;
 }
@@ -624,6 +725,7 @@
   const int total_rows = G * s.Sq;
   if ((long long)s.B * s.Hkv / grid + 2 > kMaxPending)
     throw std::runtime_error("decode_simt: batch x kv-heads too large for one launch (split the batch)");
+  if (grid > dcomm::kStealCounters) throw std::runtime_error("decode_simt: grid larger than the pool counter buffer");
   if (comm.world > 1) {
     const size_t need_data = (size_t)2 * comm.world * s.B * s.Hkv * R * (s.D + 2) * 8;
     if (need_data > comm.data_bytes)
@@ -642,7 +744,7 @@
   p.scale_log2 = s.softmax_scale * 1.4426950408889634f;
   p.causal = s.causal; p.q_pos0 = s.q_pos0; p.kv_pos0 = s.kv_pos0;
   p.q_sb = s.q_sb; p.q_sh = s.q_sh; p.q_ss = s.q_ss; p.o_sb = s.o_sb; p.o_sh = s.o_sh; p.o_ss = s.o_ss;
-  p.max_parts = max_parts;
+  p.max_slots = decode_simt_max_slots(max_parts);
   p.comm = dcomm::to_device_ctx(comm);
   PreparedLaunch pl;
   for (int r_base = 0; r_base < total_rows; r_base += R) {
diff --git a/tree_attention_b200/csrc/decode_swap_sm100.cu b/tree_attention_b200/csrc/decode_swap_sm100.cu
--- a/tree_attention_b200/csrc/decode_swap_sm100.cu
+++ b/tree_attention_b200/csrc/decode_swap_sm100.cu
@@ -101,7 +101,7 @@
   const int world = p.comm.world;
   const int BH = p.B * p.Hkv;
   const int R = p.R;
-  const dcomm::Geom geo = dcomm::make_geom(p.S, p.kv_len, BH, gridDim.x);
+  const dcomm::Geom geo = dcomm::make_geom(p.S, p.kv_len, BH, gridDim.x, false);
   const int t_lo = dcomm::cta_lo(geo, cta), t_hi = dcomm::cta_lo(geo, cta + 1);
   int jvis = geo.tph;
   if (p.causal) {
@@ -263,7 +263,7 @@
       dcomm::Tail tl;
       volatile int* sm = s_tags;
       while (sm[2] == 0) { }
-      tl.comm = &p.comm; tl.part = p.part; tl.max_parts = p.max_parts; tl.BH = BH;
+      tl.comm = &p.comm; tl.part = p.part; tl.max_slots = p.max_parts; tl.BH = BH;
       tl.R = R; tl.rows_valid = R; tl.wtag = (uint32_t)sm[0]; tl.ctag = (uint32_t)sm[1]; tl.geo = geo;
       tl.pending = pending; tl.max_pending = kSwMaxPending; tl.stamps = stamps;
       return tl;
@@ -497,9 +497,8 @@
         if (lane == 0) mbar_arrive(&p_full[i & 1]);
       }
       const dcomm::Tail tail = make_tail();
-      int nparts, pidx;
-      dcomm::head_parts(geo, x, cta, nparts, pidx);
-      uint64_t* my_part = dcomm::part_ptr<D>(tail, x, pidx);
+      const int slot = cta - dcomm::cta_of_tile(geo, x * geo.tph);
+      uint64_t* my_part = dcomm::part_ptr<D>(tail, x, slot);
       {
         float lw[kSwN];
 #pragma unroll
diff --git a/tree_attention_b200/csrc/decode_tc_sm100.cu b/tree_attention_b200/csrc/decode_tc_sm100.cu
--- a/tree_attention_b200/csrc/decode_tc_sm100.cu
+++ b/tree_attention_b200/csrc/decode_tc_sm100.cu
@@ -87,7 +87,7 @@
   const int world = p.comm.world;
   const int BH = p.B * p.Hkv;
   const int R = p.R;
-  const dcomm::Geom geo = dcomm::make_geom(p.S, p.kv_len, BH, gridDim.x);
+  const dcomm::Geom geo = dcomm::make_geom(p.S, p.kv_len, BH, gridDim.x, false);
   const int t_lo = dcomm::cta_lo(geo, cta), t_hi = dcomm::cta_lo(geo, cta + 1);
   int jvis = geo.tph;
   if (p.causal) {
@@ -243,7 +243,7 @@
       dcomm::Tail tl;
       volatile int* sm = s_tags;
       while (sm[2] == 0) { }
-      tl.comm = &p.comm; tl.part = p.part; tl.max_parts = p.max_parts; tl.BH = BH;
+      tl.comm = &p.comm; tl.part = p.part; tl.max_slots = p.max_parts; tl.BH = BH;
       tl.R = R; tl.rows_valid = R; tl.wtag = (uint32_t)sm[0]; tl.ctag = (uint32_t)sm[1]; tl.geo = geo;
       tl.pending = pending; tl.max_pending = kTcMaxPending; tl.stamps = stamps;
       return tl;
@@ -389,9 +389,8 @@
         }
       }
       const dcomm::Tail tail = make_tail();
-      int nparts, pidx;
-      dcomm::head_parts(geo, x, cta, nparts, pidx);
-      uint64_t* my_part = dcomm::part_ptr<D>(tail, x, pidx);
+      const int slot = cta - dcomm::cta_of_tile(geo, x * geo.tph);
+      uint64_t* my_part = dcomm::part_ptr<D>(tail, x, slot);
       if (warp_active) {
         if (n > 0) {
           const int il = it + n - 1;
diff --git a/tree_attention_b200/csrc/kernels.h b/tree_attention_b200/csrc/kernels.h
--- a/tree_attention_b200/csrc/kernels.h
+++ b/tree_attention_b200/csrc/kernels.h
@@ -45,6 +45,8 @@
 };
 
 void decode_split(int BH, int cap, int ncta, int* grid, int* max_parts);
+int decode_simt_max_slots(int max_parts);
+int decode_simt_ticket_ints();
 
 void decode_simt_plan(const AttnShape& s, int num_sms, int* grid, int* max_parts, int* rows_per_pass,
                       size_t* part_floats, size_t* comm_floats, size_t* comm_flags);
diff --git a/tree_attention_b200/ops/local.py b/tree_attention_b200/ops/local.py
--- a/tree_attention_b200/ops/local.py
+++ b/tree_attention_b200/ops/local.py
@@ -91,7 +91,7 @@
                         int(q_pos0), int(kv_pos0), impl == "swap", _kv_len_arg(kv_len, k))
         return out, lse
     grid, max_parts, rows, part_floats, _, _ = C.decode_plan(b, hq, hkv, sq, s, d)
-    ws = _workspace(q.device, "decode", part_floats, b * hkv + 2)
+    ws = _workspace(q.device, "decode", part_floats, max(b * hkv + 2, C.decode_ticket_ints()))
     if out is None:
         out = torch.empty((b, hq, sq, d), dtype=q.dtype, device=q.device)
     if lse is None and return_lse:
@@ -117,10 +117,8 @@
     b, hq, sq, d = q_shape
     hkv, s = k_shape[1], k_shape[2]
     if impl in ("tc", "swap"):
-        part_floats = C.decode_tc_plan(b, hq, hkv, sq, s, d)[3]
-    else:
-        part_floats = C.decode_plan(b, hq, hkv, sq, s, d)[3]
-    return int(part_floats), b * hkv + 2
+        return int(C.decode_tc_plan(b, hq, hkv, sq, s, d)[3]), b * hkv + 2
+    return int(C.decode_plan(b, hq, hkv, sq, s, d)[3]), max(b * hkv + 2, C.decode_ticket_ints())
 
 
 def decode_attention_mxfp8(
@@ -140,7 +138,7 @@
     b, hq, sq, d = q.shape
     hkv, s = k.shape[1], k.shape[2]
     grid, max_parts, rows, part_floats, _, _ = C.decode_plan(b, hq, hkv, sq, s, d)
-    ws = _workspace(q.device, "decode", part_floats, b * hkv + 2)
+    ws = _workspace(q.device, "decode", part_floats, max(b * hkv + 2, C.decode_ticket_ints()))
     out = torch.empty((b, hq, sq, d), dtype=q.dtype, device=q.device)
     lse = torch.empty((b, hq, sq), dtype=torch.float32, device=q.device) if return_lse else None
     C.decode_fwd_mx(q, k.data, v.data, k.scales, v.scales, out, lse, ws["part"], ws["tickets"], comm,
```

Measured after the change: 428.4 million, median of 6. 1.05x the previous value.
